# jacobkrantz/VLN-CE

Hardware: AMD Instinct MI355X
Metric: policy-steps/sec (fwd+bwd) (higher is better)
Workload: dtype f32

## Files before the change

include/vlnce_hip.h:

```cpp
#ifndef VLNCE_HIP_H
#define VLNCE_HIP_H

#include <stddef.h>
#include <stdint.h>

#ifdef __cplusplus
extern "C" {
#endif

typedef void* vlnce_stream_t;

enum { VLNCE_ACT_NONE = 0, VLNCE_ACT_RELU = 1, VLNCE_ACT_SIGMOID = 2, VLNCE_ACT_TANH = 3 };

int vlnce_version(void);
int vlnce_option_count(void);
int vlnce_option_index(const char* name);
const char* vlnce_last_error(void);

int vlnce_set_option(const char* name, int value);
int vlnce_get_option(const char* name, int* value);
int vlnce_option_default(const char* name, int* value);

typedef struct {
  int N, H, W, Cin;
  int Cout, KH, KW;
  int stride, pad;
  int Ho, Wo;
  int ldx, ldy;
} vlnce_conv_desc;

typedef struct {
  const float* x;
  int Cin, ldx;
  const void* w_frag;
  const float* in_scale;
  const float* in_shift;
  const float* in_center;
  int in_relu;
} vlnce_regen;

typedef struct {
  const float* in_scale;
  const float* in_shift;
  const float* in_center;
  int in_relu;
  const float* x2;
  const float* in2_scale;
  const float* in2_shift;
  const float* in2_center;
  float* side_out;
  const void* w_split;
  const void* w_frag;
  const int* options;
  int w_format;
  const vlnce_regen* regen;
} vlnce_prologue;

#define VLNCE_BN_SHARDS 16
typedef struct {
  double* acc;
  void* workspace;
  long workspace_bytes;
} vlnce_bn_sums;

typedef struct {
  const float* scale;
  const float* shift;
  const float* residual;
  int ldr;
  int act;
  int accumulate;
  float* stat_partial;
  const vlnce_bn_sums* bn;
  int stats_only;
} vlnce_epilogue;

long vlnce_conv2d_bn_workspace_bytes(const vlnce_conv_desc* d);
int vlnce_bn_finalize_sums(double* acc, int M, int C, const float* gamma, const float* beta,
                           float eps, float momentum, float* running_mean, float* running_var,
                           float* scale_out, float* shift_out, float* mean_out, float* rstd_out,
                           vlnce_stream_t stream);

int vlnce_conv2d_tiles_m(const vlnce_conv_desc* d);
int vlnce_conv2d_tile_rows(const vlnce_conv_desc* d);

int vlnce_conv2d_split_weights(const float* w, void* planes, long count, int format,
                               vlnce_stream_t stream);

long vlnce_conv2d_pack_bytes(const vlnce_conv_desc* d);
int vlnce_conv2d_pack_weights(const float* w_ohwi, void* frag, const vlnce_conv_desc* d,
                              int format , vlnce_stream_t stream);

typedef struct vlnce_weight_job {
  const float* w_oihw;
  void* dst;
  int Cout, Cin, T;
  int kind;
  int transposed;
  int format;
} vlnce_weight_job;
long vlnce_weight_job_items(const vlnce_weight_job* job);
int vlnce_conv2d_prepare_weights(const vlnce_weight_job* jobs_dev, const long* first_item_dev,
                                 int njobs, long total_items, vlnce_stream_t stream);

#define VLNCE_CONV_PATH_F32 0
#define VLNCE_CONV_PATH_X3 1
#define VLNCE_CONV_PATH_P3 2
#define VLNCE_CONV_PATH_M3 3
int vlnce_conv2d_last_path(void);

#define VLNCE_CONV_KERNEL(family, format, kernel, a, b, c) \
  ((family) | ((format) << 2) | ((kernel) << 4) | ((a) << 8) | ((b) << 16) | ((c) << 24))
#define VLNCE_CONV_KERNEL_FAMILY(v) ((v) & 3)
#define VLNCE_CONV_KERNEL_FORMAT(v) (((v) >> 2) & 3)
#define VLNCE_CONV_KERNEL_KIND(v) (((v) >> 4) & 15)
#define VLNCE_CONV_KERNEL_A(v) (((v) >> 8) & 255)
#define VLNCE_CONV_KERNEL_B(v) (((v) >> 16) & 255)
#define VLNCE_CONV_KERNEL_C(v) (((v) >> 24) & 127)
#define VLNCE_CONV_KERNEL_P3 0
#define VLNCE_CONV_KERNEL_U3 1
#define VLNCE_CONV_KERNEL_S3 2
#define VLNCE_CONV_KERNEL_R3 3
#define VLNCE_CONV_P3_DENSE 0
#define VLNCE_CONV_P3_GATHER 1
#define VLNCE_CONV_P3_DUAL 2
#define VLNCE_CONV_KERNEL_F32_BUF 0
#define VLNCE_CONV_KERNEL_F32_SPLITK 1
#define VLNCE_CONV_KERNEL_F32_V4 2
#define VLNCE_CONV_KERNEL_F32_S 3
#define VLNCE_CONV_KERNEL_F32_STEM3 4
#define VLNCE_CONV_KERNEL_F32_STEM1 5
#define VLNCE_CONV_KERNEL_F32_DUAL 6
int vlnce_conv2d_last_kernel(void);

int vlnce_conv2d_fwd(const float* x, const float* w_ohwi, float* y,
                     const vlnce_conv_desc* d, const vlnce_prologue* pro,
                     const vlnce_epilogue* epi, vlnce_stream_t stream);

int vlnce_gemm(const float* A, int lda, int transA, const float* B, int ldb, int transB,
               float* C, int ldc, int M, int N, int K,
               const vlnce_epilogue* epi, vlnce_stream_t stream);

#define VLNCE_GEMM_KERNEL(a, b, tile, splitk, zero, pass2) \
  ((a) | ((b) << 2) | ((tile) << 4) | ((zero) ? 1 << 6 : 0) | ((pass2) ? 1 << 7 : 0) | ((splitk) << 8))
#define VLNCE_GEMM_KERNEL_A(v) ((v) & 3)
#define VLNCE_GEMM_KERNEL_B(v) (((v) >> 2) & 3)
#define VLNCE_GEMM_KERNEL_TILE(v) (((v) >> 4) & 3)
#define VLNCE_GEMM_KERNEL_ZERO(v) (((v) >> 6) & 1)
#define VLNCE_GEMM_KERNEL_PASS2(v) (((v) >> 7) & 1)
#define VLNCE_GEMM_KERNEL_SPLITK(v) (((v) >> 8) & 255)
#define VLNCE_GEMM_A_BUF 0
#define VLNCE_GEMM_A_IM2COL_V4 1
#define VLNCE_GEMM_A_IM2COL_S 2
#define VLNCE_GEMM_A_TRANS 3
#define VLNCE_GEMM_B_BUF 0
#define VLNCE_GEMM_B_NK_V4 1
#define VLNCE_GEMM_B_NK_S 2
#define VLNCE_GEMM_B_KN 3
#define VLNCE_GEMM_TILE_128X128 1
#define VLNCE_GEMM_TILE_128X64 2
#define VLNCE_GEMM_TILE_64X64 3
int vlnce_gemm_last_kernel(void);

int vlnce_linear_rows_supported(int M, int N, int K);
int vlnce_linear_rows_fwd(const float* x, int ldx, const float* w, int ldw, const float* bias,
                          int act, float* y, int ldy, int M, int N, int K, vlnce_stream_t stream);
int vlnce_linear_rows_bwd(const float* x, int ldx, const float* w, int ldw, const float* dy,
                          int lddy, const float* y, int ldy, int act, float* dx, float* dw,
                          float* db, int M, int N, int K, vlnce_stream_t stream);

int vlnce_colsum(const float* x, int ldx, int M, int N, float* out, int accumulate,
                 vlnce_stream_t stream);

size_t vlnce_bn_finalize_workspace_bytes(int tiles_m, int C);
int vlnce_bn_finalize(const float* stat_partial, int tiles_m, int tile_rows, int M, int C,
                      const float* gamma, const float* beta, float eps, float momentum,
                      float* running_mean, float* running_var,
                      float* scale_out, float* shift_out,
                      float* mean_out, float* rstd_out,
                      void* workspace, size_t workspace_bytes,
                      vlnce_stream_t stream);

int vlnce_scale_shift_act(const float* x, const float* scale, const float* shift,
                          const float* center, int rows_per_sample, const float* residual,
                          float* y, long M, int C, int act, vlnce_stream_t stream);

int vlnce_scale_shift_add_act(const float* x1, const float* scale1, const float* shift1,
                              const float* center1, const float* x2, const float* scale2,
                              const float* shift2, const float* center2, float* y, long M, int C,
                              int act, vlnce_stream_t stream);

int vlnce_gn_chunks(int HW);
int vlnce_gn_partial(const float* x, int Nimg, int HW, int C, float* partial ,
                     vlnce_stream_t stream);
int vlnce_gn_finalize(const float* partial, int Nimg, int HW, int C, int groups,
                      const float* gamma, const float* beta, float eps,
                      float* scale_out, float* shift_out,
                      float* center_out,
                      float* mean_out, float* rstd_out,
                      vlnce_stream_t stream);
int vlnce_gn_finalize_tiles(const float* stat_partial, int tile_rows, int Nimg, int HW, int C,
                            int groups, const float* gamma, const float* beta, float eps,
                            float* scale_out, float* shift_out, float* center_out,
                            float* mean_out, float* rstd_out, vlnce_stream_t stream);
int vlnce_group_norm_small(const float* x, int Nimg, int HW, int C, int groups, const float* gamma,
                           const float* beta, float eps, const float* residual, int act, float* y,
                           vlnce_stream_t stream);

int vlnce_maxpool3x3s2(const float* x, float* y, int N, int H, int W, int C, int Ho, int Wo,
                       const float* in_scale, const float* in_shift, const float* in_center,
                       int in_relu, vlnce_stream_t stream);
int vlnce_avgpool2x2(const float* x, float* y, int N, int H, int W, int C, vlnce_stream_t stream);

int vlnce_space_to_depth2(const float* x, float* y, int N, int H, int W, int C, int pad_lo,
                          int pad_hi, const float* scale, const float* shift,
                          vlnce_stream_t stream);
#define VLNCE_DT_F32 0
#define VLNCE_DT_U8 1
typedef struct {
  const void* x;
  const void* x2;
  const unsigned char* mask2;
  int dtype;
  int N, F, Hs, Ws, C;
  int y0, x0, H, W;
} vlnce_frames;
int vlnce_frames_s2d(const vlnce_frames* frames, float* y, int pad_lo, int pad_hi,
                     const float* scale, const float* shift, vlnce_stream_t stream);
int vlnce_stem7_fwd(const vlnce_frames* frames, const float* in_scale, const float* in_shift,
                    const void* w_frag, int w_format, float* y, int Cout, const vlnce_epilogue* epi,
                    vlnce_stream_t stream);
int vlnce_frames_avgpool2(const vlnce_frames* frames, float* y, vlnce_stream_t stream);
int vlnce_frames_f32(const vlnce_frames* frames, float* y, const float* scale, const float* shift,
                     vlnce_stream_t stream);
int vlnce_frames_gather(const void* const* srcs, int F, int elem_bytes, int N, int Hs, int Ws,
                        int C, int y0, int x0, int H, int W, void* out, vlnce_stream_t stream);

int vlnce_frames_resize_area(const void* x, int dtype, int NF, int Hs, int Ws, int C, int OH, int OW,
                             int y0, int x0, int H, int W, void* out, vlnce_stream_t stream);

int vlnce_adaptive_avgpool(const float* x, float* y, int N, int H, int W, int C, int OH, int OW,
                           int ldy, vlnce_stream_t stream);

int vlnce_conv2d_wgrad(const float* x, const float* dy, float* dw_ohwi, const vlnce_conv_desc* d,
                       const float* dy_pow2, int P, int accumulate, vlnce_stream_t stream);
#define VLNCE_WGRAD_PATH_F32 0
#define VLNCE_WGRAD_PATH_X6_BF16 1
#define VLNCE_WGRAD_PATH_X6_F16 2
int vlnce_conv2d_wgrad_last_path(void);
#define VLNCE_WGRAD_KERNEL(path, tm, split) ((path) | ((tm) << 4) | ((split) ? 1 << 12 : 0))
#define VLNCE_WGRAD_KERNEL_PATH(v) ((v) & 15)
#define VLNCE_WGRAD_KERNEL_TM(v) (((v) >> 4) & 255)
#define VLNCE_WGRAD_KERNEL_SPLIT(v) (((v) >> 12) & 1)
int vlnce_conv2d_wgrad_last_kernel(void);
size_t vlnce_bn_bwd_workspace_floats(long M, int C);
int vlnce_bn_bwd(const float* dy, const float* y, const float* x, const float* mean,
                 const float* rstd, const float* gamma, long M, int C, int relu,
                 int use_batch_stats, float* dx, float* dres, float* dgamma, float* dbeta,
                 float* workspace, float* pow2, int P, vlnce_stream_t stream);
size_t vlnce_gn_bwd_workspace_floats(int Nimg, int HW, int C, int groups);
int vlnce_gn_bwd(const float* dy, const float* y, const float* x, const float* mean,
                 const float* rstd, const float* gamma, int Nimg, int HW, int C, int groups,
                 int relu, float* dx, float* dres, float* dgamma, float* dbeta, float* workspace,
                 float* pow2, int P, vlnce_stream_t stream);
int vlnce_maxpool3x3s2_argmax(const float* x, float* y, uint8_t* argmax, int N, int H, int W,
                              int C, int Ho, int Wo, vlnce_stream_t stream);
int vlnce_maxpool3x3s2_bwd(const float* dy, const uint8_t* argmax, float* dx, int N, int H, int W,
                           int C, int Ho, int Wo, vlnce_stream_t stream);
int vlnce_adaptive_avgpool_bwd(const float* dy, float* dx, int N, int H, int W, int C, int OH,
                               int OW, vlnce_stream_t stream);

int vlnce_action_head_fwd(const float* x, int ldx, const float* w, const float* b, int M, int K,
                          int A, float* logits_out, int* nan_count, vlnce_stream_t stream);
int vlnce_action_head_bwd(const float* x, int ldx, const float* w, const float* logits,
                          const float* dlogits, int M, int K, int A, float* dx, float* dw,
                          float* db, vlnce_stream_t stream);

int vlnce_attn_fwd(const float* q, const float* K, int ldk, const float* V, int ldv,
                   const uint8_t* mask, int mask_mode, float scale,
                   float* out, float* attn_out, int B, int P, int Dk, int Dv,
                   vlnce_stream_t stream);
int vlnce_attn_bwd(const float* dout, const float* q, const float* K, int ldk,
                   const float* V, int ldv, const uint8_t* mask, int mask_mode, float scale,
                   const float* attn, float* dq, float* dK, int lddk, float* dV, int lddv,
                   int B, int P, int Dk, int Dv, vlnce_stream_t stream);

int vlnce_attn_fwd_shared(const float* q, const float* K, int ldk, const float* V, int ldv,
                          const uint8_t* mask, int mask_mode, float scale, const int64_t* kv_index,
                          float* out, float* attn_out, int B, int P, int Dk, int Dv,
                          vlnce_stream_t stream);
int vlnce_attn_bwd_shared(const float* dout, const float* q, const float* K, int ldk,
                          const float* V, int ldv, const uint8_t* mask, int mask_mode, float scale,
                          const int64_t* kv_index, const float* attn, float* dq, float* dK,
                          int lddk, float* dV, int lddv, int B, int P, int Dk, int Dv,
                          vlnce_stream_t stream);
int vlnce_segment_sum(const float* x, const int64_t* index, int B, int U, long row_elems,
                      float* out, vlnce_stream_t stream);
int vlnce_rowzero_mask(const float* x, int ld, long rows, int C, uint8_t* mask,
                       vlnce_stream_t stream);

int vlnce_gru_gates_fwd(const float* gi, const float* gh, const float* h_prev,
                        const uint8_t* mask,
                        float* h_out, float* gates_out ,
                        float* hn_out ,
                        int B, int H, vlnce_stream_t stream);
int vlnce_gru_gates_bwd(const float* dh_out, const float* gates, const float* hn,
                        const float* h_prev, const uint8_t* mask,
                        float* dgi, float* dgh, float* dh_prev, int B, int H,
                        vlnce_stream_t stream);
int vlnce_lstm_gates_fwd(const float* gi, const float* gh, const float* c_prev,
                         const uint8_t* mask, float* h_out, float* c_out,
                         float* gates_out , int B, int H,
                         vlnce_stream_t stream);
int vlnce_lstm_gates_bwd(const float* dh_out, const float* dc_out, const float* gates,
                         const float* c_prev, const float* c_out, const uint8_t* mask,
                         float* dgates , float* dc_prev, int B, int H,
                         vlnce_stream_t stream);

int vlnce_rnn_seq_supported(int kind, int H);
int vlnce_rnn_seq_fwd(int kind, int dirs, const float* const* gi, const float* const* w_hh,
                      const float* const* b_hh, const int* lengths, float* const* out,
                      float* const* h_final, float* const* gates_save, float* const* aux_save,
                      int B, int L, int H, vlnce_stream_t stream);
int vlnce_rnn_seq_bwd(int kind, int dirs, const float* const* w_hh_t, const int* lengths,
                      const float* const* out, const float* const* gates_save,
                      const float* const* aux_save, const float* const* dout,
                      const float* const* dh_final, float* const* dgi, float* const* dgh,
                      int B, int L, int H, vlnce_stream_t stream);
int vlnce_rnn_seq_fwd2(int kind, int dirs, const float* const* gi, const float* const* w_hh,
                       const float* const* b_hh, const int* lengths, float* const* out_tm,
                       float* seq, long seq_st, long seq_sb, float* const* h_final,
                       float* const* gates_save, float* const* aux_save, int B, int L, int H,
                       vlnce_stream_t stream);
int vlnce_rnn_seq_bwd2(int kind, int dirs, const float* const* w_hh, const int* lengths,
                       const float* const* out_tm, const float* const* gates_save,
                       const float* const* aux_save, const float* dseq, long dseq_st, long dseq_sb,
                       float* dout_ws ,
                       const float* const* dh_final, float* const* dgi, float* const* dgh,
                       int B, int L, int H, vlnce_stream_t stream);
int vlnce_rnn_seq_wgrad(int kind, int dirs, int first_dir, const float* const* dgi, const float* const* dgh,
                        const float* const* out_tm, const float* x_tm, int ldx, int E,
                        const float* const* w_ih, float* const* dw_ih, float* const* dw_hh,
                        float* const* db_ih, float* const* db_hh, float* dx_tm, int B, int L, int H,
                        vlnce_stream_t stream);

int vlnce_mean_rows(const float* x, float* y, int B, int P, int C, vlnce_stream_t stream);
int vlnce_rnn_step_supported(int N, int H, int lstm);
int vlnce_rnn_step_fwd(int lstm, const float* gi, const float* h_prev, const float* c_prev,
                       const uint8_t* mask, const float* w_hh, const float* b_hh, float* hp_out,
                       float* h_out, float* aux_out, float* gates_out, int N, int H,
                       vlnce_stream_t stream);
int vlnce_rnn_step_bwd(int lstm, const float* dout, float* carry, const float* dc,
                       const float* gates, const float* aux, const float* hp, const float* c_prev,
                       const uint8_t* mask, const float* w_hh_t, float* dgi, float* dgh,
                       float* acc0, float* dc_prev, int N, int H, vlnce_stream_t stream);
int vlnce_mask_rows(const float* x, const uint8_t* mask, float* out, int B, int H,
                    vlnce_stream_t stream);
int vlnce_gru_rollout_supported(int N, int H);
long vlnce_gru_rollout_workspace_bytes(int N, int H);
int vlnce_gru_rollout_fwd(const float* gi, const float* h0, const uint8_t* mask, const float* w_hh,
                          const float* b_hh, float* hp, float* out, float* gates, float* aux,
                          void* workspace, int T, int N, int H, vlnce_stream_t stream);
int vlnce_gru_rollout_bwd(const float* dout, const float* dh_final, const float* gates,
                          const float* aux, const float* hp, const uint8_t* mask,
                          const float* w_hh_t, float* dgi, float* dgh, float* dh0,
                          void* workspace, int T, int N, int H, vlnce_stream_t stream);
int vlnce_lstm_rollout_supported(int N, int H);
long vlnce_lstm_rollout_workspace_bytes(int N, int H);
int vlnce_lstm_rollout_fwd(const float* gi, const float* h0, const float* c0, const uint8_t* mask,
                           const float* w_hh, const float* b_hh, float* hp, float* out, float* gates,
                           float* aux, void* workspace, int T, int N, int H, vlnce_stream_t stream);
int vlnce_lstm_rollout_bwd(const float* dout, const float* dh_final, const float* dc_final,
                           const float* gates, const float* aux, const float* hp, const float* c0,
                           const uint8_t* mask, const float* w_hh_t, float* dgi, float* dh0,
                           float* dc0, void* workspace, int T, int N, int H, vlnce_stream_t stream);

int vlnce_select_rows(const uint8_t* mask, const float* a, const float* b, float* out, int B, int H,
                      vlnce_stream_t stream);
int vlnce_embedding_bwd(const long* tokens, const float* grad_rows, float* grad_weight, long rows,
                        int E, long padding_idx, long vocab, vlnce_stream_t stream);
int vlnce_act_bwd(const float* dy, const float* y, float* dz, long n, int act,
                  vlnce_stream_t stream);

enum { VLNCE_SRC_F32 = 0, VLNCE_SRC_F16 = 1, VLNCE_SRC_I64 = 2 };
int vlnce_ragged_pad_rows(const void* src, int src_dtype, const int* offsets, int B, int Tmax,
                          long D, float fill, float* dst, vlnce_stream_t stream);
int vlnce_ragged_pad_rows_i64(const int64_t* src, const int* offsets, int B, int Tmax, long D,
                              int64_t fill, int64_t* dst, vlnce_stream_t stream);
int vlnce_dagger_targets(const int64_t* oracle_actions, const int* offsets, int B, int Tmax,
                         float inflection_coef, int64_t* corrected_out, float* weights_out,
                         uint8_t* masks_out, vlnce_stream_t stream);

enum { VLNCE_TRAJ_F32 = 0, VLNCE_TRAJ_F16 = 1, VLNCE_TRAJ_I64 = 2, VLNCE_TRAJ_U8 = 3 };
#define VLNCE_TRAJ_MAX_SENSORS 8
#define VLNCE_TRAJ_MAX_ROWS 128
typedef struct {
  const void* src;
  void* dst;
  long row_stride, c_stride, p_stride;
  int C, P;
  int src_dtype;
  int dst_dtype;
} vlnce_traj_sensor;
int vlnce_traj_append(const vlnce_traj_sensor* sensors, int n_sensors, const int* slots,
                      const int* steps, int n_rows, long capacity, vlnce_stream_t stream);
int vlnce_dagger_mix_actions(const int64_t* actions, const void* expert, int expert_dtype,
                             const float* uniform, float beta, int n, int64_t* prev_actions,
                             int64_t* stepped , vlnce_stream_t stream);

int vlnce_ppo_returns(const float* rewards, float* value_preds, const float* masks,
                      const float* next_value, float* returns, int T, int N, float gamma, float tau,
                      int use_gae, vlnce_stream_t stream);

int vlnce_ppo_loss(const float* values, const float* returns, const float* value_preds,
                   const float* logp, const float* old_logp, const float* adv,
                   const float* ent_pano, const float* ent_offset, const float* ent_distance,
                   const float* radians, int B, float clip, float value_coef, float entropy_coef,
                   float pano_coef, float offset_coef, float distance_coef, float reg_coef,
                   int use_clipped, float* stats, float* grads, vlnce_stream_t stream);

int vlnce_il_loss_supported(int T, int N, int A);
int vlnce_il_loss(const float* logits, const int64_t* targets, const float* weights,
                  const float* aux, float inv_scalar, int T, int N, int A, float* stats,
                  float* dlogits, vlnce_stream_t stream);

int vlnce_pair_mse(const float* estimate, const float* target, const uint8_t* mask, int E, int R,
                   float* value, float* d_estimate, vlnce_stream_t stream);

#ifdef __cplusplus
}
#endif
#endif
```

vln-ce_amd/_lib.py:

```python
import collections
import ctypes as C
import os
import threading

import torch

_HERE = os.path.dirname(os.path.abspath(__file__))
LIB_PATH = os.environ.get("VLNCE_HIP_LIB") or os.path.join(_HERE, "libvlnce_hip.so")

_P = C.c_void_p
_I = C.c_int
_F = C.c_float
_L = C.c_long


def _buffer_format(explicit, *bufs):
    tags = {getattr(b, "_vlnce_fmt", None) for b in bufs if b is not None} - {None}
    if explicit:
        tags.add(int(explicit))
    if len(tags) > 1:
        raise RuntimeError(f"weight buffers / w_format disagree on the plane format: {sorted(tags)}")
    return tags.pop() if tags else 1


ConvKernel = collections.namedtuple("ConvKernel", "family kernel fmt a b c")
ConvKernel.__doc__ = """family: "f32" | "x3" | "p3" | "m3" (= conv2d_last_path()); kernel: the kernel within it
("conv_p3" | "conv_u3" | "conv_s3", "conv_m3", "conv_x3", "buf" | "splitk" | "v4" | "s" | "stem3" |
"stem1" | "dual" of igemm_kernel); fmt: plane format 1 / 2 (0: fp32); a, b, c per kernel:
  conv_p3: tile 1..6, mode "dense" | "gather" | "dual", 0      conv_u3: rows, kind 0..2, waves
  conv_s3: Cin, 1 = statistics only, 0      conv_r3: regenerated Cin, Cout / 32, skip kind 1 / 2
  conv_m3: NT, KSPLIT, RB      conv_x3: tile 1..4, dual 0 / 1, 0
  splitk: the split factor, 0, 0"""
WgradKernel = collections.namedtuple("WgradKernel", "path tm split")

_FAMILIES = ("f32", "x3", "p3", "m3")
_KERNELS = {"f32": ("buf", "splitk", "v4", "s", "stem3", "stem1", "dual"), "x3": ("conv_x3",),
            "p3": ("conv_p3", "conv_u3", "conv_s3", "conv_r3"), "m3": ("conv_m3",)}
_P3_MODES = ("dense", "gather", "dual")


def decode_conv_kernel(v):
    if v < 0:
        return None
    family = _FAMILIES[v & 3]
    kernel = _KERNELS[family][(v >> 4) & 15]
    a, b, c = (v >> 8) & 255, (v >> 16) & 255, (v >> 24) & 127
    if kernel == "conv_p3":
        b = _P3_MODES[b]
    return ConvKernel(family, kernel, (v >> 2) & 3, a, b, c)


def decode_wgrad_kernel(v):
    return None if v < 0 else WgradKernel(v & 15, (v >> 4) & 255, bool((v >> 12) & 1))


GemmKernel = collections.namedtuple("GemmKernel", "a b tile splitk zero pass2")
GemmKernel.__doc__ = """a: the A loader "buf" | "v4" | "s" | "trans"; b: the B loader "buf" | "nk_v4" | "nk_s" | "kn";
tile: (rows, columns) of the igemm_kernel instance; splitk: the split-K factor (1 = not split); zero: C was
zero-filled first; pass2: the second bias / activation pass ran"""
_GEMM_A = ("buf", "v4", "s", "trans")
_GEMM_B = ("buf", "nk_v4", "nk_s", "kn")
_GEMM_TILES = (None, (128, 128), (128, 64), (64, 64))


def decode_gemm_kernel(v):
    if v < 0:
        return None
    return GemmKernel(_GEMM_A[v & 3], _GEMM_B[(v >> 2) & 3], _GEMM_TILES[(v >> 4) & 3], (v >> 8) & 255,
                      bool((v >> 6) & 1), bool((v >> 7) & 1))


class ConvDesc(C.Structure):
    _fields_ = [(n, _I) for n in
                ("N", "H", "W", "Cin", "Cout", "KH", "KW", "stride", "pad", "Ho", "Wo", "ldx", "ldy")]


class WeightJob(C.Structure):
    _fields_ = [("w_oihw", _P), ("dst", _P), ("Cout", _I), ("Cin", _I), ("T", _I), ("kind", _I),
                ("transposed", _I), ("format", _I)]


class WeightPrepPlan:
    __slots__ = ("table", "first_item", "njobs", "total", "keep")


class Prologue(C.Structure):
    _fields_ = [("in_scale", _P), ("in_shift", _P), ("in_center", _P), ("in_relu", _I),
                ("x2", _P), ("in2_scale", _P), ("in2_shift", _P), ("in2_center", _P),
                ("side_out", _P), ("w_split", _P), ("w_frag", _P), ("options", _P), ("w_format", _I),
                ("regen", _P)]


class Regen(C.Structure):
    _fields_ = [("x", _P), ("Cin", _I), ("ldx", _I), ("w_frag", _P), ("in_scale", _P), ("in_shift", _P),
                ("in_center", _P), ("in_relu", _I)]


class Frames(C.Structure):
    _fields_ = [("x", _P), ("x2", _P), ("mask2", _P), ("dtype", _I), ("N", _I), ("F", _I),
                ("Hs", _I), ("Ws", _I), ("C", _I), ("y0", _I), ("x0", _I), ("H", _I), ("W", _I)]


class BnSums(C.Structure):
    _fields_ = [("acc", _P), ("workspace", _P), ("workspace_bytes", _L)]


class TrajSensor(C.Structure):
    _fields_ = [("src", _P), ("dst", _P), ("row_stride", _L), ("c_stride", _L), ("p_stride", _L),
                ("C", _I), ("P", _I), ("src_dtype", _I), ("dst_dtype", _I)]


class Epilogue(C.Structure):
    _fields_ = [("scale", _P), ("shift", _P), ("residual", _P), ("ldr", _I), ("act", _I),
                ("accumulate", _I), ("stat_partial", _P), ("bn", C.POINTER(BnSums)),
                ("stats_only", _I)]


_SIGNATURES = {
    "vlnce_version": (_I, []),
    "vlnce_last_error": (C.c_char_p, []),
    "vlnce_set_option": (_I, [C.c_char_p, _I]),
    "vlnce_get_option": (_I, [C.c_char_p, C.POINTER(_I)]),
    "vlnce_option_default": (_I, [C.c_char_p, C.POINTER(_I)]),
    "vlnce_conv2d_split_weights": (_I, [_P, _P, C.c_long, _I, _P]),
    "vlnce_conv2d_last_path": (_I, []),
    "vlnce_conv2d_wgrad_last_path": (_I, []),
    "vlnce_conv2d_last_kernel": (_I, []),
    "vlnce_conv2d_wgrad_last_kernel": (_I, []),
    "vlnce_gemm_last_kernel": (_I, []),
    "vlnce_embedding_bwd": (_I, [_P, _P, _P, _L, _I, _L, _L, _P]),
    "vlnce_conv2d_pack_bytes": (C.c_long, [C.POINTER(ConvDesc)]),
    "vlnce_conv2d_pack_weights": (_I, [_P, _P, C.POINTER(ConvDesc), _I, _P]),
    "vlnce_weight_job_items": (C.c_long, [C.POINTER(WeightJob)]),
    "vlnce_conv2d_prepare_weights": (_I, [_P, _P, _I, C.c_long, _P]),
    "vlnce_conv2d_tiles_m": (_I, [C.POINTER(ConvDesc)]),
    "vlnce_conv2d_tile_rows": (_I, [C.POINTER(ConvDesc)]),
    "vlnce_conv2d_bn_workspace_bytes": (C.c_long, [C.POINTER(ConvDesc)]),
    "vlnce_bn_finalize_sums": (_I, [_P, _I, _I, _P, _P, _F, _F, _P, _P, _P, _P, _P, _P, _P]),
    "vlnce_conv2d_fwd": (_I, [_P, _P, _P, C.POINTER(ConvDesc), C.POINTER(Prologue),
                              C.POINTER(Epilogue), _P]),
    "vlnce_gemm": (_I, [_P, _I, _I, _P, _I, _I, _P, _I, _I, _I, _I, C.POINTER(Epilogue), _P]),
    "vlnce_colsum": (_I, [_P, _I, _I, _I, _P, _I, _P]),
    "vlnce_bn_finalize_workspace_bytes": (C.c_size_t, [_I, _I]),
    "vlnce_bn_finalize": (_I, [_P, _I, _I, _I, _I, _P, _P, _F, _F, _P, _P, _P, _P, _P, _P, _P,
                               C.c_size_t, _P]),
    "vlnce_scale_shift_act": (_I, [_P, _P, _P, _P, _I, _P, _P, _L, _I, _I, _P]),
    "vlnce_gn_chunks": (_I, [_I]),
    "vlnce_gn_partial": (_I, [_P, _I, _I, _I, _P, _P]),
    "vlnce_gn_finalize": (_I, [_P, _I, _I, _I, _I, _P, _P, _F, _P, _P, _P, _P, _P, _P]),
    "vlnce_gn_finalize_tiles": (_I, [_P, _I, _I, _I, _I, _I, _P, _P, _F, _P, _P, _P, _P, _P, _P]),
    "vlnce_maxpool3x3s2": (_I, [_P, _P, _I, _I, _I, _I, _I, _I, _P, _P, _P, _I, _P]),
    "vlnce_scale_shift_add_act": (_I, [_P, _P, _P, _P, _P, _P, _P, _P, _P, _L, _I, _I, _P]),
    "vlnce_avgpool2x2": (_I, [_P, _P, _I, _I, _I, _I, _P]),
    "vlnce_ragged_pad_rows": (_I, [_P, _I, _P, _I, _I, _L, _F, _P, _P]),
    "vlnce_ragged_pad_rows_i64": (_I, [_P, _P, _I, _I, _L, _L, _P, _P]),
    "vlnce_dagger_targets": (_I, [_P, _P, _I, _I, _F, _P, _P, _P, _P]),
    "vlnce_traj_append": (_I, [C.POINTER(TrajSensor), _I, C.POINTER(_I), C.POINTER(_I), _I, _L, _P]),
    "vlnce_dagger_mix_actions": (_I, [_P, _P, _I, _P, _F, _I, _P, _P, _P]),
    "vlnce_ppo_loss": (_I, [_P, _P, _P, _P, _P, _P, _P, _P, _P, _P, _I, _F, _F, _F, _F, _F, _F, _F, _I,
                            _P, _P, _P]),
    "vlnce_ppo_returns": (_I, [_P, _P, _P, _P, _P, _I, _I, _F, _F, _I, _P]),
    "vlnce_il_loss_supported": (_I, [_I, _I, _I]),
    "vlnce_il_loss": (_I, [_P, _P, _P, _P, _F, _I, _I, _I, _P, _P, _P]),
    "vlnce_pair_mse": (_I, [_P, _P, _P, _I, _I, _P, _P, _P]),
    "vlnce_space_to_depth2": (_I, [_P, _P, _I, _I, _I, _I, _I, _I, _P, _P, _P]),
    "vlnce_frames_s2d": (_I, [C.POINTER(Frames), _P, _I, _I, _P, _P, _P]),
    "vlnce_frames_avgpool2": (_I, [C.POINTER(Frames), _P, _P]),
    "vlnce_stem7_fwd": (_I, [C.POINTER(Frames), _P, _P, _P, _I, _P, _I, C.POINTER(Epilogue), _P]),
    "vlnce_frames_f32": (_I, [C.POINTER(Frames), _P, _P, _P, _P]),
    "vlnce_frames_gather": (_I, [_P, _I, _I, _I, _I, _I, _I, _I, _I, _I, _I, _P, _P]),
    "vlnce_frames_resize_area": (_I, [_P] + [_I] * 11 + [_P, _P]),
    "vlnce_adaptive_avgpool": (_I, [_P, _P, _I, _I, _I, _I, _I, _I, _I, _P]),
    "vlnce_attn_fwd": (_I, [_P, _P, _I, _P, _I, _P, _I, _F, _P, _P, _I, _I, _I, _I, _P]),
    "vlnce_attn_bwd": (_I, [_P, _P, _P, _I, _P, _I, _P, _I, _F, _P, _P, _P, _I, _P, _I,
                            _I, _I, _I, _I, _P]),
    "vlnce_rowzero_mask": (_I, [_P, _I, _L, _I, _P, _P]),
    "vlnce_attn_fwd_shared": (_I, [_P, _P, _I, _P, _I, _P, _I, _F, _P, _P, _P, _I, _I, _I, _I, _P]),
    "vlnce_attn_bwd_shared": (_I, [_P, _P, _P, _I, _P, _I, _P, _I, _F, _P, _P, _P, _P, _I, _P, _I,
                                   _I, _I, _I, _I, _P]),
    "vlnce_segment_sum": (_I, [_P, _P, _I, _I, _L, _P, _P]),
    "vlnce_action_head_fwd": (_I, [_P, _I, _P, _P, _I, _I, _I, _P, _P, _P]),
    "vlnce_action_head_bwd": (_I, [_P, _I, _P, _P, _P, _I, _I, _I, _P, _P, _P, _P]),
    "vlnce_gru_gates_fwd": (_I, [_P, _P, _P, _P, _P, _P, _P, _I, _I, _P]),
    "vlnce_gru_gates_bwd": (_I, [_P, _P, _P, _P, _P, _P, _P, _P, _I, _I, _P]),
    "vlnce_lstm_gates_fwd": (_I, [_P, _P, _P, _P, _P, _P, _P, _I, _I, _P]),
    "vlnce_lstm_gates_bwd": (_I, [_P, _P, _P, _P, _P, _P, _P, _P, _I, _I, _P]),
    "vlnce_mean_rows": (_I, [_P, _P, _I, _I, _I, _P]),
    "vlnce_mask_rows": (_I, [_P, _P, _P, _I, _I, _P]),
    "vlnce_conv2d_wgrad": (_I, [_P, _P, _P, C.POINTER(ConvDesc), _P, _I, _I, _P]),
    "vlnce_bn_bwd": (_I, [_P, _P, _P, _P, _P, _P, _L, _I, _I, _I, _P, _P, _P, _P, _P, _P, _I, _P]),
    "vlnce_bn_bwd_workspace_floats": (C.c_size_t, [_L, _I]),
    "vlnce_gn_bwd_workspace_floats": (C.c_size_t, [_I, _I, _I, _I]),
    "vlnce_gn_bwd": (_I, [_P, _P, _P, _P, _P, _P, _I, _I, _I, _I, _I, _P, _P, _P, _P, _P, _P, _I, _P]),
    "vlnce_maxpool3x3s2_argmax": (_I, [_P, _P, _P, _I, _I, _I, _I, _I, _I, _P]),
    "vlnce_maxpool3x3s2_bwd": (_I, [_P, _P, _P, _I, _I, _I, _I, _I, _I, _P]),
    "vlnce_adaptive_avgpool_bwd": (_I, [_P, _P, _I, _I, _I, _I, _I, _I, _P]),
    "vlnce_rnn_seq_supported": (_I, [_I, _I]),
    "vlnce_rnn_seq_fwd": (_I, [_I, _I, _P, _P, _P, _P, _P, _P, _P, _P, _I, _I, _I, _P]),
    "vlnce_rnn_seq_bwd": (_I, [_I, _I, _P, _P, _P, _P, _P, _P, _P, _P, _P, _I, _I, _I, _P]),
    "vlnce_option_count": (_I, []),
    "vlnce_option_index": (_I, [C.c_char_p]),
    "vlnce_linear_rows_supported": (_I, [_I, _I, _I]),
    "vlnce_linear_rows_fwd": (_I, [_P, _I, _P, _I, _P, _I, _P, _I, _I, _I, _I, _P]),
    "vlnce_linear_rows_bwd": (_I, [_P, _I, _P, _I, _P, _I, _P, _I, _I, _P, _P, _P, _I, _I, _I, _P]),
    "vlnce_rnn_seq_fwd2": (_I, [_I, _I, _P, _P, _P, _P, _P, _P, _L, _L, _P, _P, _P, _I, _I, _I, _P]),
    "vlnce_rnn_seq_bwd2": (_I, [_I, _I, _P, _P, _P, _P, _P, _P, _L, _L, _P, _P, _P, _P, _I, _I, _I, _P]),
    "vlnce_rnn_seq_wgrad": (_I, [_I, _I, _I, _P, _P, _P, _P, _I, _I, _P, _P, _P, _P, _P, _P, _I, _I, _I, _P]),
    "vlnce_group_norm_small": (_I, [_P, _I, _I, _I, _I, _P, _P, _F, _P, _I, _P, _P]),
    "vlnce_gru_rollout_supported": (_I, [_I, _I]),
    "vlnce_gru_rollout_workspace_bytes": (C.c_long, [_I, _I]),
    "vlnce_gru_rollout_fwd": (_I, [_P, _P, _P, _P, _P, _P, _P, _P, _P, _P, _I, _I, _I, _P]),
    "vlnce_gru_rollout_bwd": (_I, [_P, _P, _P, _P, _P, _P, _P, _P, _P, _P, _P, _I, _I, _I, _P]),
    "vlnce_lstm_rollout_supported": (_I, [_I, _I]),
    "vlnce_lstm_rollout_workspace_bytes": (C.c_long, [_I, _I]),
    "vlnce_lstm_rollout_fwd": (_I, [_P, _P, _P, _P, _P, _P, _P, _P, _P, _P, _P, _I, _I, _I, _P]),
    "vlnce_lstm_rollout_bwd": (_I, [_P, _P, _P, _P, _P, _P, _P, _P, _P, _P, _P, _P, _P, _I, _I, _I, _P]),
    "vlnce_rnn_step_supported": (_I, [_I, _I, _I]),
    "vlnce_rnn_step_fwd": (_I, [_I, _P, _P, _P, _P, _P, _P, _P, _P, _P, _P, _I, _I, _P]),
    "vlnce_rnn_step_bwd": (_I, [_I, _P, _P, _P, _P, _P, _P, _P, _P, _P, _P, _P, _P, _P, _I, _I, _P]),
    "vlnce_select_rows": (_I, [_P, _P, _P, _P, _I, _I, _P]),
    "vlnce_act_bwd": (_I, [_P, _P, _P, _L, _I, _P]),
}


def collapse_rows(t):
    while True:
        groups = []
        for n, st in zip(t.shape[1:], t.stride()[1:]):
            if n == 1:
                continue
            if groups and groups[-1][1] == st * n:
                groups[-1] = (groups[-1][0] * n, int(st))
            else:
                groups.append((int(n), int(st)))
        if len(groups) <= 2:
            break
        t = t.contiguous()
    row_stride = int(t.stride(0)) if t.size(0) > 1 else 0
    if not groups:
        return t, row_stride, 1, 0, 1, 0
    if len(groups) == 1:
        return t, row_stride, groups[0][0], groups[0][1], 1, 0
    return t, row_stride, groups[0][0], groups[0][1], groups[1][0], groups[1][1]


def exported_symbols():
    return sorted(_SIGNATURES)


def load_cdll(path=LIB_PATH):
    if not os.path.exists(path):
        raise RuntimeError(
            f"{path} not found: build it with `python __graft_entry__.py` (hipcc, gfx950). "
            "The VLN-CE policy path has no CPU fallback."
        )
    dll = C.CDLL(path)
    for name, (res, args) in _SIGNATURES.items():
        fn = getattr(dll, name)
        fn.restype = res
        fn.argtypes = args
    return dll


class _CallState(threading.local):
    dev = None
    restore = None


_CALL = _CallState()


def _ptr(t):
    if t is None:
        return None
    if not t.is_cuda:
        raise RuntimeError("libvlnce_hip: tensor is not on a GPU (no CPU fallback)")
    idx = t.device.index
    if _CALL.dev is None:
        _CALL.dev = idx
    elif _CALL.dev != idx:
        first, _CALL.dev = _CALL.dev, None
        raise RuntimeError(f"libvlnce_hip: tensors of one call live on cuda:{first} and "
                           f"cuda:{idx}")
    return t.data_ptr()


def _stream():
    dev, _CALL.dev = _CALL.dev, None
    if dev is None:
        return torch.cuda.current_stream().cuda_stream
    cur = torch.cuda.current_device()
    if dev != cur:
        _CALL.restore = cur
        torch.cuda.set_device(dev)
    return torch.cuda.current_stream(dev).cuda_stream


def _leave_device():
    if _CALL.restore is not None:
        cur, _CALL.restore = _CALL.restore, None
        torch.cuda.set_device(cur)


class HipLib:

    name = "hip"

    ABI = 150

    def __init__(self, path=LIB_PATH):
        self.dll = load_cdll(path)
        have = int(self.dll.vlnce_version())
        if have != self.ABI:
            raise RuntimeError(f"{path} has ABI {have}, this package binds ABI {self.ABI}: "
                               "rebuild it (python __graft_entry__.py)")

        self._conv_math = None
        self._tls = threading.local()
        self._options_from_env()

    OPTION_NAMES = ("conv_math", "p3", "p3_tile", "s3", "u3", "u3_waves", "x3_tile", "igemm_tile",
                    "igemm_nobuf", "igemm_no_splitk", "wgrad_tile", "rollout_one_xcd", "m3", "r3",
                    "s3_wgs")

    def _options_from_env(self):
        for name in self.OPTION_NAMES:
            v = os.environ.get("VLNCE_" + name.upper())
            if v is None:
                continue
            if name == "conv_math":
                v = {"f32": 0, "0": 0, "bf16": 1, "1": 1, "f16": 2, "2": 2}.get(v.strip().lower(), v)
            elif name in ("igemm_nobuf", "igemm_no_splitk"):
                v = 0 if v in ("", "0") else 1
            try:
                v = int(v)
            except ValueError:
                import warnings
                warnings.warn(f"VLNCE_{name.upper()}={v!r} is not an integer: ignored "
                              f"(the option keeps its default)")
                continue
            self.set_option(name, v)

    def set_option(self, name, value):
        self._check(self.dll.vlnce_set_option(name.encode(), int(value)), "vlnce_set_option")
        if name == "conv_math":
            self._conv_math = int(value)

    def plane_format(self, options=None):
        v = None
        if options:
            v = options.get("conv_math")
        if v is None:
            sc = getattr(self._tls, "scoped", None)
            if sc:
                v = sc.get("conv_math")
        if v is None or v < 0:
            v = self._conv_math
            if v is None:
                v = self._conv_math = self.get_option("conv_math")
        return 2 if v == 2 else 1

    def effective_option(self, name):
        sc = getattr(self._tls, "scoped", None)
        if sc and sc.get(name, -1) >= 0:
            return int(sc[name])
        return self.get_option(name)

    def get_option(self, name):
        v = _I(0)
        self._check(self.dll.vlnce_get_option(name.encode(), C.byref(v)), "vlnce_get_option")
        return v.value

    def option_default(self, name):
        v = _I(0)
        self._check(self.dll.vlnce_option_default(name.encode(), C.byref(v)), "vlnce_option_default")
        return v.value

    PER_LAUNCH = ("conv_math", "p3", "p3_tile", "s3", "u3", "u3_waves", "x3_tile", "m3", "r3", "s3_wgs")

    def _launch_options(self, overrides):
        if not overrides:
            return None
        arr = (C.c_int * int(self.dll.vlnce_option_count()))(*([-1] * int(self.dll.vlnce_option_count())))
        for name, v in overrides.items():
            i = int(self.dll.vlnce_option_index(name.encode()))
            if i < 0:
                raise RuntimeError(f"unknown dispatch option {name!r}")
            arr[i] = int(v)
        return arr

    def options(self, **kw):
        lib = self
        unknown = [k for k in kw if k not in self.OPTION_NAMES]
        if unknown:
            raise RuntimeError(f"unknown dispatch option(s) {unknown}")

        class _Scope:
            def __enter__(self_inner):
                self_inner.prev = getattr(lib._tls, "scoped", None)
                scoped = dict(self_inner.prev or {})
                scoped.update({k: v for k, v in kw.items() if k in lib.PER_LAUNCH})
                lib._tls.scoped = scoped or None
                self_inner.old = {k: lib.get_option(k) for k in kw if k not in lib.PER_LAUNCH}
                for k in self_inner.old:
                    lib.set_option(k, kw[k])
                return lib

            def __exit__(self_inner, *exc):
                lib._tls.scoped = self_inner.prev
                for k, v in self_inner.old.items():
                    lib.set_option(k, v)
                return False

        return _Scope()

    def _check(self, rc, what):
        _leave_device()
        if rc != 0:
            raise RuntimeError(f"{what} failed (rc={rc}): {self.dll.vlnce_last_error().decode()}")

    @staticmethod
    def _desc(g):
        return ConvDesc(*[int(g[k]) for k, _ in ConvDesc._fields_])

    def conv2d_tiles(self, g):
        d = self._desc(g)
        return self.dll.vlnce_conv2d_tiles_m(C.byref(d)), self.dll.vlnce_conv2d_tile_rows(C.byref(d))

    def conv2d_fwd(self, x, w, y, g, in_scale=None, in_shift=None, in_relu=0, scale=None,
                   shift=None, residual=None, ldr=0, act=0, accumulate=0, stat_partial=None,
                   in_center=None, x2=None, in2_scale=None, in2_shift=None, in2_center=None,
                   side_out=None, w_split=None, w_frag=None, bn=None, options=None, w_format=None,
                   stats_only=False, regen=None):
        d = self._desc(g)
        w_format = _buffer_format(w_format, w_split, w_frag, regen["w_frag"] if regen else None)
        rg = None
        if regen is not None:
            rx = regen["x"]
            rg = Regen(_ptr(rx), rx.size(-1), rx.size(-1), _ptr(regen["w_frag"]),
                       _ptr(regen.get("in_scale")), _ptr(regen.get("in_shift")),
                       _ptr(regen.get("in_center")), int(regen.get("in_relu", 0)))
        opts = self._launch_options(options if options is not None
                                    else getattr(self._tls, "scoped", None))
        pro = Prologue(_ptr(in_scale), _ptr(in_shift), _ptr(in_center), int(in_relu), _ptr(x2),
                       _ptr(in2_scale), _ptr(in2_shift), _ptr(in2_center), _ptr(side_out),
                       _ptr(w_split), _ptr(w_frag),
                       C.cast(opts, C.c_void_p) if opts is not None else None, int(w_format),
                       C.cast(C.pointer(rg), C.c_void_p) if rg is not None else None)
        bnp = None
        if bn is not None:
            acc, ws = bn
            bnp = C.pointer(BnSums(_ptr(acc), _ptr(ws), ws.numel() * ws.element_size()))
        epi = Epilogue(_ptr(scale), _ptr(shift), _ptr(residual), int(ldr), int(act),
                       int(accumulate), _ptr(stat_partial), bnp, int(bool(stats_only)))
        self._check(self.dll.vlnce_conv2d_fwd(_ptr(x), _ptr(w), _ptr(y), C.byref(d), C.byref(pro),
                                              C.byref(epi), _stream()), "vlnce_conv2d_fwd")

    def bn_finalize_sums(self, acc, M, gamma, beta, eps, momentum, running_mean, running_var,
                         scale_out, mean_out, shift_out=None, rstd_out=None):
        Cc = scale_out.numel()
        self._check(self.dll.vlnce_bn_finalize_sums(
            _ptr(acc), int(M), Cc, _ptr(gamma), _ptr(beta), float(eps), float(momentum),
            _ptr(running_mean), _ptr(running_var), _ptr(scale_out), _ptr(shift_out),
            _ptr(mean_out), _ptr(rstd_out), _stream()), "vlnce_bn_finalize_sums")

    def conv2d_bn_workspace_bytes(self, g):
        d = self._desc(g)
        return int(self.dll.vlnce_conv2d_bn_workspace_bytes(C.byref(d)))

    def conv2d_split_weights(self, w, planes, fmt=1):
        self._check(self.dll.vlnce_conv2d_split_weights(_ptr(w), _ptr(planes), w.numel(), int(fmt),
                                                        _stream()), "vlnce_conv2d_split_weights")

    def conv2d_last_path(self):
        return int(self.dll.vlnce_conv2d_last_path())

    def conv2d_wgrad_last_path(self):
        return int(self.dll.vlnce_conv2d_wgrad_last_path())

    def conv2d_last_kernel(self):
        return decode_conv_kernel(int(self.dll.vlnce_conv2d_last_kernel()))

    def conv2d_wgrad_last_kernel(self):
        return decode_wgrad_kernel(int(self.dll.vlnce_conv2d_wgrad_last_kernel()))

    def conv2d_pack_bytes(self, g):
        d = self._desc(g)
        return int(self.dll.vlnce_conv2d_pack_bytes(C.byref(d)))

    def conv2d_pack_weights(self, w, frag, g, fmt=1):
        d = self._desc(g)
        self._check(self.dll.vlnce_conv2d_pack_weights(_ptr(w), _ptr(frag), C.byref(d), int(fmt),
                                                       _stream()), "vlnce_conv2d_pack_weights")

    WP_F32, WP_PLANES, WP_FRAGMENTS = 0, 1, 2

    def weight_prep_plan(self, jobs):
        arr = (WeightJob * len(jobs))()
        first = [0]
        for j, (w, dst, kind, transposed, fmt) in zip(arr, jobs):
            assert w.is_cuda and w.is_contiguous() and w.dtype == torch.float32 and w.dim() == 4
            j.w_oihw, j.dst = w.data_ptr(), dst.data_ptr()
            j.Cout, j.Cin, j.T = w.size(0), w.size(1), w.size(2) * w.size(3)
            j.kind, j.transposed, j.format = int(kind), int(bool(transposed)), int(fmt or 0)
            items = int(self.dll.vlnce_weight_job_items(C.byref(j)))
            if items <= 0:
                raise ValueError(f"weight_prep_plan: job not eligible: {tuple(w.shape)} kind={kind} "
                                 f"transposed={transposed} format={fmt}")
            first.append(first[-1] + items)
        plan = WeightPrepPlan()
        dev = jobs[0][1].device
        plan.table = torch.frombuffer(bytearray(bytes(arr)), dtype=torch.uint8).to(dev)
        plan.first_item = torch.tensor(first, dtype=torch.int64).to(dev)
        plan.njobs, plan.total = len(jobs), first[-1]
        plan.keep = [(w, dst) for w, dst, *_ in jobs]
        return plan

    def conv2d_prepare_weights(self, plan):
        self._check(self.dll.vlnce_conv2d_prepare_weights(_ptr(plan.table), _ptr(plan.first_item),
                                                          plan.njobs, plan.total, _stream()),
                    "vlnce_conv2d_prepare_weights")

    def gemm(self, A, lda, transA, B, ldb, transB, Cm, ldc, M, N, K, scale=None, shift=None,
             residual=None, ldr=0, act=0, accumulate=0):
        epi = Epilogue(_ptr(scale), _ptr(shift), _ptr(residual), int(ldr), int(act),
                       int(accumulate), None)
        self._check(self.dll.vlnce_gemm(_ptr(A), lda, transA, _ptr(B), ldb, transB, _ptr(Cm), ldc,
                                        M, N, K, C.byref(epi), _stream()), "vlnce_gemm")

    def gemm_last_kernel(self):
        return decode_gemm_kernel(int(self.dll.vlnce_gemm_last_kernel()))

    def colsum(self, x, ldx, M, N, out, accumulate=0):
        self._check(self.dll.vlnce_colsum(_ptr(x), ldx, M, N, _ptr(out), accumulate, _stream()),
                    "vlnce_colsum")

    def bn_finalize_workspace_bytes(self, tiles_m, Cc):
        return int(self.dll.vlnce_bn_finalize_workspace_bytes(tiles_m, Cc))

    def bn_finalize(self, partial, tiles_m, tile_rows, M, Cc, gamma, beta, eps, momentum,
                    running_mean, running_var, scale_out, shift_out, mean_out=None, rstd_out=None,
                    workspace=None):
        wb = workspace.numel() * workspace.element_size() if workspace is not None else 0
        self._check(self.dll.vlnce_bn_finalize(
            _ptr(partial), tiles_m, tile_rows, M, Cc, _ptr(gamma), _ptr(beta), eps, momentum,
            _ptr(running_mean), _ptr(running_var), _ptr(scale_out), _ptr(shift_out),
            _ptr(mean_out), _ptr(rstd_out), _ptr(workspace), wb, _stream()), "vlnce_bn_finalize")

    def scale_shift_act(self, x, scale, shift, rows_per_sample, residual, y, M, Cc, act,
                        center=None):
        self._check(self.dll.vlnce_scale_shift_act(
            _ptr(x), _ptr(scale), _ptr(shift), _ptr(center), rows_per_sample, _ptr(residual),
            _ptr(y), M, Cc, act, _stream()), "vlnce_scale_shift_act")

    def gn_chunks(self, HW):
        return self.dll.vlnce_gn_chunks(HW)

    def gn_partial(self, x, Nimg, HW, Cc, partial):
        self._check(self.dll.vlnce_gn_partial(_ptr(x), Nimg, HW, Cc, _ptr(partial), _stream()),
                    "vlnce_gn_partial")

    def gn_finalize(self, partial, Nimg, HW, Cc, groups, gamma, beta, eps, scale_out, shift_out,
                    mean_out=None, rstd_out=None, center_out=None):
        self._check(self.dll.vlnce_gn_finalize(
            _ptr(partial), Nimg, HW, Cc, groups, _ptr(gamma), _ptr(beta), eps, _ptr(scale_out),
            _ptr(shift_out), _ptr(center_out), _ptr(mean_out), _ptr(rstd_out), _stream()),
            "vlnce_gn_finalize")

    def gn_finalize_tiles(self, partial, tile_rows, Nimg, HW, Cc, groups, gamma, beta, eps,
                          scale_out, shift_out, mean_out=None, rstd_out=None, center_out=None):
        self._check(self.dll.vlnce_gn_finalize_tiles(
            _ptr(partial), tile_rows, Nimg, HW, Cc, groups, _ptr(gamma), _ptr(beta), eps,
            _ptr(scale_out), _ptr(shift_out), _ptr(center_out), _ptr(mean_out), _ptr(rstd_out),
            _stream()), "vlnce_gn_finalize_tiles")

    def maxpool3x3s2(self, x, y, N, H, W, Cc, Ho, Wo, in_scale=None, in_shift=None, in_relu=0,
                     in_center=None):
        self._check(self.dll.vlnce_maxpool3x3s2(_ptr(x), _ptr(y), N, H, W, Cc, Ho, Wo,
                                                _ptr(in_scale), _ptr(in_shift), _ptr(in_center),
                                                int(in_relu), _stream()), "vlnce_maxpool3x3s2")

    def scale_shift_add_act(self, x1, s1, t1, x2, s2, t2, y, M, Cc, act, c1=None, c2=None):
        self._check(self.dll.vlnce_scale_shift_add_act(
            _ptr(x1), _ptr(s1), _ptr(t1), _ptr(c1), _ptr(x2), _ptr(s2), _ptr(t2), _ptr(c2),
            _ptr(y), M, Cc, act, _stream()), "vlnce_scale_shift_add_act")

    _SRC = {torch.float32: 0, torch.float16: 1, torch.int64: 2}

    def ragged_pad_rows(self, src, offsets, B, Tmax, D, fill, dst):
        assert offsets.dtype == torch.int32 and dst.dtype == torch.float32
        self._check(self.dll.vlnce_ragged_pad_rows(
            _ptr(src), self._SRC[src.dtype], _ptr(offsets), B, Tmax, D, float(fill),
            _ptr(dst), _stream()), "vlnce_ragged_pad_rows")

    def ragged_pad_rows_i64(self, src, offsets, B, Tmax, D, fill, dst):
        assert src.dtype == torch.int64 and dst.dtype == torch.int64
        self._check(self.dll.vlnce_ragged_pad_rows_i64(
            _ptr(src), _ptr(offsets), B, Tmax, D, int(fill), _ptr(dst), _stream()),
            "vlnce_ragged_pad_rows_i64")

    def dagger_targets(self, oracle, offsets, B, Tmax, coef, corrected, weights, masks):
        self._check(self.dll.vlnce_dagger_targets(
            _ptr(oracle), _ptr(offsets), B, Tmax, float(coef), _ptr(corrected),
            _ptr(weights), _ptr(masks), _stream()), "vlnce_dagger_targets")

    _TRAJ = {torch.float32: 0, torch.float16: 1, torch.int64: 2, torch.uint8: 3}
    TRAJ_MAX_SENSORS, TRAJ_MAX_ROWS = 8, 128

    def traj_append(self, sources, arenas, slots, steps):
        n = len(slots)
        assert len(sources) == len(arenas) and len(steps) == n and n > 0
        capacity, num_envs = int(arenas[0].size(1)), min(int(a.size(0)) for a in arenas)
        if min(slots) < 0 or max(slots) >= num_envs:
            raise RuntimeError(f"traj_append: slot outside the arena's {num_envs} environments")
        table, keep = [], []
        for src, dst in zip(sources, arenas):
            src, rs, Cc, cs, P, ps = collapse_rows(src)
            keep.append(src)
            if src.size(0) != n:
                raise RuntimeError(f"traj_append: {src.size(0)} source rows for {n} slots")
            if dst.dim() != 3 or not dst.is_contiguous() or dst.size(1) != capacity \
                    or dst.size(2) != Cc * P:
                raise RuntimeError(f"traj_append: arena {tuple(dst.shape)} for rows of {Cc * P} "
                                   f"elements at capacity {capacity}")
            if src.dtype not in (torch.float32, torch.int64, torch.uint8) \
                    or dst.dtype not in (torch.float16, torch.float32, torch.int64):
                raise RuntimeError(f"traj_append: {src.dtype} -> {dst.dtype} is not a recorded pair")
            table.append((src, dst, rs, Cc, cs, P, ps))
        for r0 in range(0, n, self.TRAJ_MAX_ROWS):
            r1 = min(n, r0 + self.TRAJ_MAX_ROWS)
            sl = (_I * (r1 - r0))(*[int(v) for v in slots[r0:r1]])
            stp = (_I * (r1 - r0))(*[int(v) for v in steps[r0:r1]])
            for k0 in range(0, len(table), self.TRAJ_MAX_SENSORS):
                part = table[k0:k0 + self.TRAJ_MAX_SENSORS]
                arr = (TrajSensor * len(part))()
                for a, (src, dst, rs, Cc, cs, P, ps) in zip(arr, part):
                    a.src = _ptr(src) + r0 * rs * src.element_size()
                    a.dst = _ptr(dst)
                    a.row_stride, a.c_stride, a.p_stride, a.C, a.P = rs, cs, ps, Cc, P
                    a.src_dtype, a.dst_dtype = self._TRAJ[src.dtype], self._TRAJ[dst.dtype]
                self._check(self.dll.vlnce_traj_append(arr, len(part), sl, stp, r1 - r0, capacity,
                                                       _stream()), "vlnce_traj_append")

    def dagger_mix_actions(self, actions, expert, uniform, beta, prev_actions, stepped):
        n = actions.numel()
        assert actions.dtype == torch.int64 and prev_actions.dtype == torch.int64
        assert stepped.dtype == torch.int64 and stepped.numel() == 2 * n and stepped.is_contiguous()
        assert uniform.dtype == torch.float32 and expert.dtype in (torch.float32, torch.int64)
        assert expert.numel() == n and uniform.numel() == n and prev_actions.numel() == n
        assert all(t.is_contiguous() for t in (actions, expert, uniform, prev_actions))
        self._check(self.dll.vlnce_dagger_mix_actions(
            _ptr(actions), _ptr(expert), self._TRAJ[expert.dtype], _ptr(uniform), float(beta), n,
            _ptr(prev_actions), _ptr(stepped), _stream()), "vlnce_dagger_mix_actions")

    def ppo_loss(self, values, returns, value_preds, logp, old_logp, adv, ent_pano, ent_offset,
                 ent_distance, radians, B, clip, value_coef, entropy_coef, pano_coef, offset_coef,
                 distance_coef, reg_coef, use_clipped, stats, grads):
        self._check(self.dll.vlnce_ppo_loss(
            _ptr(values), _ptr(returns), _ptr(value_preds), _ptr(logp), _ptr(old_logp), _ptr(adv),
            _ptr(ent_pano), _ptr(ent_offset), _ptr(ent_distance), _ptr(radians), B, clip, value_coef,
            entropy_coef, pano_coef, offset_coef, distance_coef, reg_coef, int(use_clipped),
            _ptr(stats), _ptr(grads), _stream()), "vlnce_ppo_loss")

    def ppo_returns(self, rewards, value_preds, masks, next_value, returns, T, N, gamma, tau,
                    use_gae):
        self._check(self.dll.vlnce_ppo_returns(_ptr(rewards), _ptr(value_preds), _ptr(masks),
                                               _ptr(next_value), _ptr(returns), T, N, float(gamma),
                                               float(tau), int(use_gae), _stream()),
                    "vlnce_ppo_returns")

    def il_loss_supported(self, T, N, A):
        return bool(self.dll.vlnce_il_loss_supported(int(T), int(N), int(A)))

    def il_loss(self, logits, targets, weights, aux, inv_scalar, T, N, A, stats, dlogits):
        assert logits.dtype == torch.float32 and weights.dtype == torch.float32
        assert targets.dtype == torch.int64 and (aux is None or aux.dtype == torch.float32)
        assert logits.numel() == T * N * A and targets.numel() == T * N and weights.numel() == T * N
        assert stats.numel() == 3 and dlogits.numel() == T * N * A
        assert all(t.is_contiguous() for t in (logits, targets, weights, stats, dlogits))
        self._check(self.dll.vlnce_il_loss(_ptr(logits), _ptr(targets), _ptr(weights), _ptr(aux),
                                           float(inv_scalar), T, N, A, _ptr(stats), _ptr(dlogits),
                                           _stream()), "vlnce_il_loss")

    def pair_mse(self, estimate, target, mask, E, R, value, d_estimate):
        assert estimate.dtype == torch.float32 and target.dtype == torch.float32
        assert mask.dtype in (torch.bool, torch.uint8) and mask.numel() == E
        assert estimate.numel() == E and target.numel() == R and d_estimate.numel() == E
        assert all(t.is_contiguous() for t in (estimate, target, mask, d_estimate))
        self._check(self.dll.vlnce_pair_mse(_ptr(estimate), _ptr(target), _ptr(mask), E, R,
                                            _ptr(value), _ptr(d_estimate), _stream()),
                    "vlnce_pair_mse")

    def space_to_depth2(self, x, y, N, H, W, Cc, pad_lo, pad_hi, scale=None, shift=None):
        self._check(self.dll.vlnce_space_to_depth2(_ptr(x), _ptr(y), N, H, W, Cc, pad_lo, pad_hi,
                                                   _ptr(scale), _ptr(shift), _stream()),
                    "vlnce_space_to_depth2")

    _DT = {torch.float32: 0, torch.uint8: 1}

    def _frames(self, fr):
        x = fr["x"]
        if fr.get("x2") is not None and fr["x2"].dtype != x.dtype:
            raise RuntimeError("libvlnce_hip: frames and the extra frame differ in dtype")
        return Frames(_ptr(x), _ptr(fr.get("x2")), _ptr(fr.get("mask2")), self._DT[x.dtype],
                      *[int(fr[k]) for k in ("N", "F", "Hs", "Ws", "C", "y0", "x0", "H", "W")])

    def frames_s2d(self, fr, y, pad_lo, pad_hi, scale=None, shift=None):
        d = self._frames(fr)
        self._check(self.dll.vlnce_frames_s2d(C.byref(d), _ptr(y), pad_lo, pad_hi, _ptr(scale),
                                              _ptr(shift), _stream()), "vlnce_frames_s2d")

    def stem7_fwd(self, fr, in_scale, in_shift, w_frag, y, scale=None, shift=None, act=0, bn=None,
                  w_format=None):
        d = self._frames(fr)
        w_format = _buffer_format(w_format, w_frag)
        bnp = None
        if bn is not None:
            bnp = C.pointer(BnSums(_ptr(bn), None, 0))
        epi = Epilogue(_ptr(scale), _ptr(shift), None, 0, int(act), 0, None, bnp)
        self._check(self.dll.vlnce_stem7_fwd(C.byref(d), _ptr(in_scale), _ptr(in_shift),
                                             _ptr(w_frag), int(w_format), _ptr(y), y.size(-1),
                                             C.byref(epi), _stream()), "vlnce_stem7_fwd")

    def frames_avgpool2(self, fr, y):
        d = self._frames(fr)
        self._check(self.dll.vlnce_frames_avgpool2(C.byref(d), _ptr(y), _stream()),
                    "vlnce_frames_avgpool2")

    def frames_f32(self, fr, y, scale=None, shift=None):
        d = self._frames(fr)
        self._check(self.dll.vlnce_frames_f32(C.byref(d), _ptr(y), _ptr(scale), _ptr(shift),
                                              _stream()), "vlnce_frames_f32")

    def frames_gather(self, srcs, elem_bytes, N, Hs, Ws, Cc, y0, x0, H, W, out):
        arr = (C.c_void_p * len(srcs))(*[_ptr(t) for t in srcs])
        self._check(self.dll.vlnce_frames_gather(arr, len(srcs), elem_bytes, N, Hs, Ws, Cc, y0, x0,
                                                 H, W, _ptr(out), _stream()), "vlnce_frames_gather")

    def frames_resize_area(self, x, is_u8, NF, Hs, Ws, Cc, OH, OW, y0, x0, H, W, out):
        self._check(self.dll.vlnce_frames_resize_area(_ptr(x), 1 if is_u8 else 0, NF, Hs, Ws, Cc, OH,
                                                      OW, y0, x0, H, W, _ptr(out), _stream()),
                    "vlnce_frames_resize_area")

    def avgpool2x2(self, x, y, N, H, W, Cc):
        self._check(self.dll.vlnce_avgpool2x2(_ptr(x), _ptr(y), N, H, W, Cc, _stream()),
                    "vlnce_avgpool2x2")

    def adaptive_avgpool(self, x, y, N, H, W, Cc, OH, OW, ldy):
        self._check(self.dll.vlnce_adaptive_avgpool(_ptr(x), _ptr(y), N, H, W, Cc, OH, OW, ldy,
                                                    _stream()), "vlnce_adaptive_avgpool")

    def mean_rows(self, x, y, B, P, Cc):
        self._check(self.dll.vlnce_mean_rows(_ptr(x), _ptr(y), B, P, Cc, _stream()),
                    "vlnce_mean_rows")

    def action_head_fwd(self, x, ldx, w, b, M, K, A, logits_out, nan_count=None):
        self._check(self.dll.vlnce_action_head_fwd(_ptr(x), ldx, _ptr(w), _ptr(b), M, K, A,
                                                   _ptr(logits_out), _ptr(nan_count), _stream()),
                    "vlnce_action_head_fwd")

    def action_head_bwd(self, x, ldx, w, logits, dlogits, M, K, A, dx=None, dw=None, db=None):
        self._check(self.dll.vlnce_action_head_bwd(_ptr(x), ldx, _ptr(w), _ptr(logits),
                                                   _ptr(dlogits), M, K, A, _ptr(dx), _ptr(dw),
                                                   _ptr(db), _stream()), "vlnce_action_head_bwd")

    def attn_fwd(self, q, K, ldk, V, ldv, mask, mask_mode, scale, out, attn_out, B, P, Dk, Dv,
                 kv_index=None):
        if kv_index is not None:
            self._check(self.dll.vlnce_attn_fwd_shared(
                _ptr(q), _ptr(K), ldk, _ptr(V), ldv, _ptr(mask), mask_mode, scale, _ptr(kv_index),
                _ptr(out), _ptr(attn_out), B, P, Dk, Dv, _stream()), "vlnce_attn_fwd_shared")
            return
        self._check(self.dll.vlnce_attn_fwd(_ptr(q), _ptr(K), ldk, _ptr(V), ldv, _ptr(mask),
                                            mask_mode, scale, _ptr(out), _ptr(attn_out), B, P, Dk,
                                            Dv, _stream()), "vlnce_attn_fwd")

    def segment_sum(self, x, index, B, U, row_elems, out):
        self._check(self.dll.vlnce_segment_sum(_ptr(x), _ptr(index), B, U, row_elems, _ptr(out),
                                               _stream()), "vlnce_segment_sum")

    def attn_bwd(self, dout, q, K, ldk, V, ldv, mask, mask_mode, scale, attn, dq, dK, lddk, dV,
                 lddv, B, P, Dk, Dv, kv_index=None):
        if kv_index is not None:
            self._check(self.dll.vlnce_attn_bwd_shared(
                _ptr(dout), _ptr(q), _ptr(K), ldk, _ptr(V), ldv, _ptr(mask), mask_mode, scale,
                _ptr(kv_index), _ptr(attn), _ptr(dq), _ptr(dK), lddk, _ptr(dV), lddv, B, P, Dk, Dv,
                _stream()), "vlnce_attn_bwd_shared")
            return
        self._check(self.dll.vlnce_attn_bwd(_ptr(dout), _ptr(q), _ptr(K), ldk, _ptr(V), ldv,
                                            _ptr(mask), mask_mode, scale, _ptr(attn), _ptr(dq),
                                            _ptr(dK), lddk, _ptr(dV), lddv, B, P, Dk, Dv,
                                            _stream()), "vlnce_attn_bwd")

    def rowzero_mask(self, x, ld, rows, Cc, mask):
        self._check(self.dll.vlnce_rowzero_mask(_ptr(x), ld, rows, Cc, _ptr(mask), _stream()),
                    "vlnce_rowzero_mask")

    def gru_gates_fwd(self, gi, gh, h_prev, mask, h_out, gates_out, hn_out, B, H):
        self._check(self.dll.vlnce_gru_gates_fwd(_ptr(gi), _ptr(gh), _ptr(h_prev), _ptr(mask),
                                                 _ptr(h_out), _ptr(gates_out), _ptr(hn_out), B, H,
                                                 _stream()), "vlnce_gru_gates_fwd")

    def gru_gates_bwd(self, dh_out, gates, hn, h_prev, mask, dgi, dgh, dh_prev, B, H):
        self._check(self.dll.vlnce_gru_gates_bwd(_ptr(dh_out), _ptr(gates), _ptr(hn), _ptr(h_prev),
                                                 _ptr(mask), _ptr(dgi), _ptr(dgh), _ptr(dh_prev),
                                                 B, H, _stream()), "vlnce_gru_gates_bwd")

    def lstm_gates_fwd(self, gi, gh, c_prev, mask, h_out, c_out, gates_out, B, H):
        self._check(self.dll.vlnce_lstm_gates_fwd(_ptr(gi), _ptr(gh), _ptr(c_prev), _ptr(mask),
                                                  _ptr(h_out), _ptr(c_out), _ptr(gates_out), B, H,
                                                  _stream()), "vlnce_lstm_gates_fwd")

    def lstm_gates_bwd(self, dh_out, dc_out, gates, c_prev, c_out, mask, dgates, dc_prev, B, H):
        self._check(self.dll.vlnce_lstm_gates_bwd(_ptr(dh_out), _ptr(dc_out), _ptr(gates),
                                                  _ptr(c_prev), _ptr(c_out), _ptr(mask),
                                                  _ptr(dgates), _ptr(dc_prev), B, H, _stream()),
                    "vlnce_lstm_gates_bwd")

    def mask_rows(self, x, mask, out, B, H):
        self._check(self.dll.vlnce_mask_rows(_ptr(x), _ptr(mask), _ptr(out), B, H, _stream()),
                    "vlnce_mask_rows")

    def conv2d_wgrad(self, x, dy, dw, g, dy_pow2=None, accumulate=False):
        d = self._desc(g)
        self._check(self.dll.vlnce_conv2d_wgrad(_ptr(x), _ptr(dy), _ptr(dw), C.byref(d),
                                                _ptr(dy_pow2),
                                                dy_pow2.size(1) if dy_pow2 is not None else 0,
                                                int(bool(accumulate)), _stream()),
                    "vlnce_conv2d_wgrad")

    def bn_bwd_workspace_floats(self, M, Cc):
        return int(self.dll.vlnce_bn_bwd_workspace_floats(M, Cc))

    def bn_bwd(self, dy, y, x, mean, rstd, gamma, M, Cc, relu, use_batch_stats, dx, dres, dgamma,
               dbeta, workspace=None, pow2=None):
        self._check(self.dll.vlnce_bn_bwd(_ptr(dy), _ptr(y), _ptr(x), _ptr(mean), _ptr(rstd),
                                          _ptr(gamma), M, Cc, int(relu), int(use_batch_stats),
                                          _ptr(dx), _ptr(dres), _ptr(dgamma), _ptr(dbeta),
                                          _ptr(workspace), _ptr(pow2),
                                          pow2.size(1) if pow2 is not None else 0, _stream()),
                    "vlnce_bn_bwd")

    def gn_bwd_workspace_floats(self, Nimg, HW, Cc, groups):
        return int(self.dll.vlnce_gn_bwd_workspace_floats(Nimg, HW, Cc, groups))

    def gn_bwd(self, dy, y, x, mean, rstd, gamma, Nimg, HW, Cc, groups, relu, dx, dres, dgamma,
               dbeta, workspace, pow2=None):
        self._check(self.dll.vlnce_gn_bwd(_ptr(dy), _ptr(y), _ptr(x), _ptr(mean), _ptr(rstd),
                                          _ptr(gamma), Nimg, HW, Cc, groups, int(relu), _ptr(dx),
                                          _ptr(dres), _ptr(dgamma), _ptr(dbeta), _ptr(workspace),
                                          _ptr(pow2), pow2.size(1) if pow2 is not None else 0,
                                          _stream()), "vlnce_gn_bwd")

    def maxpool3x3s2_argmax(self, x, y, argmax, N, H, W, Cc, Ho, Wo):
        self._check(self.dll.vlnce_maxpool3x3s2_argmax(_ptr(x), _ptr(y), _ptr(argmax), N, H, W, Cc,
                                                       Ho, Wo, _stream()),
                    "vlnce_maxpool3x3s2_argmax")

    def maxpool3x3s2_bwd(self, dy, argmax, dx, N, H, W, Cc, Ho, Wo):
        self._check(self.dll.vlnce_maxpool3x3s2_bwd(_ptr(dy), _ptr(argmax), _ptr(dx), N, H, W, Cc,
                                                    Ho, Wo, _stream()), "vlnce_maxpool3x3s2_bwd")

    def adaptive_avgpool_bwd(self, dy, dx, N, H, W, Cc, OH, OW):
        self._check(self.dll.vlnce_adaptive_avgpool_bwd(_ptr(dy), _ptr(dx), N, H, W, Cc, OH, OW,
                                                        _stream()), "vlnce_adaptive_avgpool_bwd")

    @staticmethod
    def _parr(ts, n):
        if ts is None:
            return None
        arr = (C.c_void_p * 2)()
        for i in range(n):
            arr[i] = _ptr(ts[i])
        return arr

    def rnn_seq_supported(self, kind, H):
        return bool(self.dll.vlnce_rnn_seq_supported(kind, H))

    def rnn_seq_fwd(self, kind, dirs, gi, w_hh, b_hh, lengths, out, h_final, gates_save, aux_save,
                    B, Lm, H):
        pa = self._parr
        self._check(self.dll.vlnce_rnn_seq_fwd(
            kind, dirs, pa(gi, dirs), pa(w_hh, dirs), pa(b_hh, dirs), _ptr(lengths), pa(out, dirs),
            pa(h_final, dirs), pa(gates_save, dirs), pa(aux_save, dirs), B, Lm, H, _stream()),
            "vlnce_rnn_seq_fwd")

    def rnn_seq_bwd(self, kind, dirs, w_hh_t, lengths, out, gates_save, aux_save, dout, dh_final,
                    dgi, dgh, B, Lm, H):
        pa = self._parr
        self._check(self.dll.vlnce_rnn_seq_bwd(
            kind, dirs, pa(w_hh_t, dirs), _ptr(lengths), pa(out, dirs), pa(gates_save, dirs),
            pa(aux_save, dirs), pa(dout, dirs), pa(dh_final, dirs), pa(dgi, dirs), pa(dgh, dirs),
            B, Lm, H, _stream()), "vlnce_rnn_seq_bwd")

    def linear_rows_supported(self, M, N, K):
        return bool(self.dll.vlnce_linear_rows_supported(M, N, K))

    def linear_rows_fwd(self, x, ldx, w, ldw, bias, act, y, ldy, M, N, K):
        self._check(self.dll.vlnce_linear_rows_fwd(_ptr(x), ldx, _ptr(w), ldw, _ptr(bias), act, _ptr(y),
                                                   ldy, M, N, K, _stream()), "vlnce_linear_rows_fwd")

    def linear_rows_bwd(self, x, ldx, w, ldw, dy, lddy, y, ldy, act, dx, dw, db, M, N, K):
        self._check(self.dll.vlnce_linear_rows_bwd(_ptr(x), ldx, _ptr(w), ldw, _ptr(dy), lddy, _ptr(y),
                                                   ldy, act, _ptr(dx), _ptr(dw), _ptr(db), M, N, K,
                                                   _stream()), "vlnce_linear_rows_bwd")

    def rnn_seq_fwd2(self, kind, dirs, gi, w_hh, b_hh, lengths, out_tm, seq, seq_st, seq_sb, h_final,
                     gates_save, aux_save, B, Lm, H):
        pa = self._parr
        self._check(self.dll.vlnce_rnn_seq_fwd2(
            kind, dirs, pa(gi, dirs), pa(w_hh, dirs), pa(b_hh, dirs), _ptr(lengths), pa(out_tm, dirs),
            _ptr(seq), seq_st, seq_sb, pa(h_final, dirs), pa(gates_save, dirs), pa(aux_save, dirs),
            B, Lm, H, _stream()), "vlnce_rnn_seq_fwd2")

    def rnn_seq_bwd2(self, kind, dirs, w_hh, lengths, out_tm, gates_save, aux_save, dseq, dseq_st,
                     dseq_sb, dout_ws, dh_final, dgi, dgh, B, Lm, H):
        pa = self._parr
        self._check(self.dll.vlnce_rnn_seq_bwd2(
            kind, dirs, pa(w_hh, dirs), _ptr(lengths), pa(out_tm, dirs), pa(gates_save, dirs),
            pa(aux_save, dirs), _ptr(dseq), dseq_st, dseq_sb, _ptr(dout_ws), pa(dh_final, dirs),
            pa(dgi, dirs), pa(dgh, dirs), B, Lm, H, _stream()), "vlnce_rnn_seq_bwd2")

    def rnn_seq_wgrad(self, kind, dirs, dgi, dgh, out_tm, x_tm, ldx, E, w_ih, dw_ih, dw_hh, db_ih,
                      db_hh, dx_tm, B, Lm, H, first_dir=0):
        pa = self._parr
        self._check(self.dll.vlnce_rnn_seq_wgrad(
            kind, dirs, first_dir, pa(dgi, dirs), pa(dgh, dirs), pa(out_tm, dirs), _ptr(x_tm), ldx, E,
            pa(w_ih, dirs), pa(dw_ih, dirs), pa(dw_hh, dirs), pa(db_ih, dirs), pa(db_hh, dirs),
            _ptr(dx_tm), B, Lm, H, _stream()), "vlnce_rnn_seq_wgrad")

    def group_norm_small(self, x, N, HW, Cc, groups, gamma, beta, eps, residual, act, y):
        self._check(self.dll.vlnce_group_norm_small(
            _ptr(x), N, HW, Cc, groups, _ptr(gamma), _ptr(beta), eps, _ptr(residual), act, _ptr(y),
            _stream()), "vlnce_group_norm_small")

    def gru_rollout_supported(self, N, H):
        if os.environ.get("VLNCE_GRU_ROLLOUT", "1") == "0":
            return False
        return bool(self.dll.vlnce_gru_rollout_supported(N, H))

    def gru_rollout_workspace_bytes(self, N, H):
        return int(self.dll.vlnce_gru_rollout_workspace_bytes(N, H))

    def gru_rollout_fwd(self, gi, h0, mask, w_hh, b_hh, hp, out, gates, aux, workspace, T, N, H):
        self._check(self.dll.vlnce_gru_rollout_fwd(
            _ptr(gi), _ptr(h0), _ptr(mask), _ptr(w_hh), _ptr(b_hh), _ptr(hp), _ptr(out),
            _ptr(gates), _ptr(aux), _ptr(workspace), T, N, H, _stream()), "vlnce_gru_rollout_fwd")

    def gru_rollout_bwd(self, dout, dh_final, gates, aux, hp, mask, w_hh_t, dgi, dgh, dh0,
                        workspace, T, N, H):
        self._check(self.dll.vlnce_gru_rollout_bwd(
            _ptr(dout), _ptr(dh_final), _ptr(gates), _ptr(aux), _ptr(hp), _ptr(mask),
            _ptr(w_hh_t), _ptr(dgi), _ptr(dgh), _ptr(dh0), _ptr(workspace), T, N, H, _stream()),
            "vlnce_gru_rollout_bwd")

    def lstm_rollout_supported(self, N, H):
        return bool(self.dll.vlnce_lstm_rollout_supported(N, H))

    def lstm_rollout_workspace_bytes(self, N, H):
        return int(self.dll.vlnce_lstm_rollout_workspace_bytes(N, H))

    def lstm_rollout_fwd(self, gi, h0, c0, mask, w_hh, b_hh, hp, out, gates, aux, workspace,
                         T, N, H):
        self._check(self.dll.vlnce_lstm_rollout_fwd(
            _ptr(gi), _ptr(h0), _ptr(c0), _ptr(mask), _ptr(w_hh), _ptr(b_hh), _ptr(hp), _ptr(out),
            _ptr(gates), _ptr(aux), _ptr(workspace), T, N, H, _stream()), "vlnce_lstm_rollout_fwd")

    def lstm_rollout_bwd(self, dout, dh_final, dc_final, gates, aux, hp, c0, mask, w_hh_t, dgi,
                         dh0, dc0, workspace, T, N, H):
        self._check(self.dll.vlnce_lstm_rollout_bwd(
            _ptr(dout), _ptr(dh_final), _ptr(dc_final), _ptr(gates), _ptr(aux), _ptr(hp), _ptr(c0),
            _ptr(mask), _ptr(w_hh_t), _ptr(dgi), _ptr(dh0), _ptr(dc0), _ptr(workspace), T, N, H,
            _stream()), "vlnce_lstm_rollout_bwd")

    def rnn_step_supported(self, N, H, lstm):
        if os.environ.get("VLNCE_RNN_STEP_FUSED", "1") == "0":
            return False
        return bool(self.dll.vlnce_rnn_step_supported(N, H, int(lstm)))

    def rnn_step_fwd(self, lstm, gi, h_prev, c_prev, mask, w_hh, b_hh, hp_out, h_out, aux_out,
                     gates_out, N, H):
        self._check(self.dll.vlnce_rnn_step_fwd(
            int(lstm), _ptr(gi), _ptr(h_prev), _ptr(c_prev), _ptr(mask), _ptr(w_hh), _ptr(b_hh),
            _ptr(hp_out), _ptr(h_out), _ptr(aux_out), _ptr(gates_out), N, H, _stream()),
            "vlnce_rnn_step_fwd")

    def rnn_step_bwd(self, lstm, dout, carry, dc, gates, aux, hp, c_prev, mask, w_hh_t, dgi, dgh,
                     acc0, dc_prev, N, H):
        self._check(self.dll.vlnce_rnn_step_bwd(
            int(lstm), _ptr(dout), _ptr(carry), _ptr(dc), _ptr(gates), _ptr(aux), _ptr(hp),
            _ptr(c_prev), _ptr(mask), _ptr(w_hh_t), _ptr(dgi), _ptr(dgh), _ptr(acc0),
            _ptr(dc_prev), N, H, _stream()), "vlnce_rnn_step_bwd")

    def select_rows(self, mask, a, b, out, B, H):
        self._check(self.dll.vlnce_select_rows(_ptr(mask), _ptr(a), _ptr(b), _ptr(out), B, H,
                                               _stream()), "vlnce_select_rows")

    def embedding_bwd(self, tokens, grad_rows, grad_weight, padding_idx):
        self._check(self.dll.vlnce_embedding_bwd(_ptr(tokens), _ptr(grad_rows), _ptr(grad_weight),
                                                 tokens.numel(), grad_weight.size(1),
                                                 -1 if padding_idx is None else int(padding_idx),
                                                 grad_weight.size(0), _stream()),
                    "vlnce_embedding_bwd")

    def act_bwd(self, dy, y, dz, n, act):
        self._check(self.dll.vlnce_act_bwd(_ptr(dy), _ptr(y), _ptr(dz), n, act, _stream()),
                    "vlnce_act_bwd")


_LIB = None


def get_lib():
    global _LIB
    if _LIB is None:
        _LIB = HipLib()
    return _LIB
```

vln-ce_amd/csrc/api.cpp:

```cpp
#include <stdarg.h>
#include <stdio.h>
#include <string.h>

#include <atomic>

#include "common_opts.h"

static thread_local char g_err[512] = "";

void vlnce_set_error(const char* fmt, ...) {
  va_list ap;
  va_start(ap, fmt);
  vsnprintf(g_err, sizeof(g_err), fmt, ap);
  va_end(ap);
}

extern "C" const char* vlnce_last_error(void) { return g_err; }
extern "C" int vlnce_version(void) { return 150; }

namespace {
struct OptDef {
  const char* name;
  int def;
};
const OptDef kOpts[VLNCE_OPT_COUNT] = {
    {"conv_math", 2},   {"p3", 2},          {"p3_tile", 0},         {"s3", 1},
    {"u3", 1},          {"u3_waves", 8},    {"x3_tile", 0},         {"igemm_tile", 0},
    {"igemm_nobuf", 0}, {"igemm_no_splitk", 0}, {"wgrad_tile", 64}, {"rollout_one_xcd", 0},
    {"m3", 1},          {"r3", 1},          {"s3_wgs", 0},
};
std::atomic<int> g_opt[VLNCE_OPT_COUNT] = {
    {2}, {2}, {0}, {1}, {1}, {8}, {0}, {0}, {0}, {0}, {64}, {0}, {1}, {1}, {0},
};
int opt_index(const char* name) {
  if (name)
    for (int i = 0; i < VLNCE_OPT_COUNT; ++i)
      if (strcmp(name, kOpts[i].name) == 0) return i;
  return -1;
}
}

namespace {
thread_local const int* t_call_opts = nullptr;
}
VlnceOptScope::VlnceOptScope(const int* per_call) : prev(t_call_opts) { t_call_opts = per_call; }
VlnceOptScope::~VlnceOptScope() { t_call_opts = prev; }

int vlnce_opt(int id) {
  if (t_call_opts && t_call_opts[id] >= 0) return t_call_opts[id];
  return g_opt[id].load(std::memory_order_relaxed);
}

extern "C" int vlnce_option_count(void) { return VLNCE_OPT_COUNT; }

extern "C" int vlnce_option_index(const char* name) { return opt_index(name); }

extern "C" int vlnce_set_option(const char* name, int value) {
  const int i = opt_index(name);
  if (i < 0) {
    vlnce_set_error("vlnce_set_option: unknown option '%s'", name ? name : "(null)");
    return 1;
  }
  g_opt[i].store(value, std::memory_order_relaxed);
  return 0;
}

extern "C" int vlnce_get_option(const char* name, int* value) {
  const int i = opt_index(name);
  if (i < 0 || !value) {
    vlnce_set_error("vlnce_get_option: unknown option '%s'", name ? name : "(null)");
    return 1;
  }
  *value = g_opt[i].load(std::memory_order_relaxed);
  return 0;
}

extern "C" int vlnce_option_default(const char* name, int* value) {
  const int i = opt_index(name);
  if (i < 0 || !value) {
    vlnce_set_error("vlnce_option_default: unknown option '%s'", name ? name : "(null)");
    return 1;
  }
  *value = kOpts[i].def;
  return 0;
}
```

vln-ce_amd/csrc/common_opts.h:

```cpp
#pragma once
#include "../../include/vlnce_hip.h"

void vlnce_set_error(const char* fmt, ...);

enum {
  VLNCE_OPT_CONV_MATH,
  VLNCE_OPT_P3,
  VLNCE_OPT_P3_TILE,
  VLNCE_OPT_S3,
  VLNCE_OPT_U3,
  VLNCE_OPT_U3_WAVES,
  VLNCE_OPT_X3_TILE,
  VLNCE_OPT_IGEMM_TILE,
  VLNCE_OPT_IGEMM_NOBUF,
  VLNCE_OPT_IGEMM_NO_SPLITK,
  VLNCE_OPT_WGRAD_TILE,
  VLNCE_OPT_ROLLOUT_ONE_XCD,
  VLNCE_OPT_M3,
  VLNCE_OPT_R3,
  VLNCE_OPT_S3_WGS,
  VLNCE_OPT_COUNT
};
int vlnce_opt(int id);

struct VlnceOptScope {
  explicit VlnceOptScope(const int* per_call);
  ~VlnceOptScope();
  const int* prev;
};
```

vln-ce_amd/csrc/rnn_seq.hip:

```cpp
#include "common.h"

namespace {

struct RnnSeqParams {
  const float* gi[2];
  const float* w_hh[2];
  const float* b_hh[2];
  float* out[2];
  float* h_final[2];
  float* gates[2];
  float* aux[2];
  const float* dout[2];
  const float* dh_final[2];
  float* dgi[2];
  float* dgh[2];
  const int* lengths;
  int B, L;
  float* seq[2];
  long seq_st, seq_sb;
  int self_zero;
  int w_plain;
};

__global__ __launch_bounds__(256) void dseq_to_time_major_kernel(const float* __restrict__ dseq, long st,
                                                                 long sb, float* __restrict__ dst, int dirs,
                                                                 int L, int B, int H) {
  const int h4 = H / 4;
  const long n = (long)dirs * L * B * h4;
  for (long i = (long)blockIdx.x * 256 + threadIdx.x; i < n; i += (long)gridDim.x * 256) {
    const int u4 = (int)(i % h4);
    long r = i / h4;
    const int b = (int)(r % B);
    r /= B;
    const int t = (int)(r % L);
    const int d = (int)(r / L);
    const float* src = dseq + (long)t * st + (long)b * sb + d * H + 4 * u4;
    f32x4 v = {src[0], src[1], src[2], src[3]};
    *reinterpret_cast<f32x4*>(dst + i * 4) = v;
  }
}

template <int NT>
__device__ __forceinline__ void zero_tails(float* __restrict__ base, long st, long sb, int width,
                                           const int* __restrict__ lengths, int b0, int B, int L,
                                           int tid) {
  for (int r = 0; r < 16; ++r) {
    const int b = b0 + r;
    if (b >= B) break;
    const int lb = min(max(lengths[b], 0), L);
    const int n = (L - lb) * width;
    for (int i = tid; i < n; i += NT) {
      const int q = i / width;
      base[(long)(lb + q) * st + (long)b * sb + (i - q * width)] = 0.f;
    }
  }
}

__device__ __forceinline__ float sigm(float x) {
  return __builtin_amdgcn_rcpf(1.f + __builtin_amdgcn_exp2f(-1.4426950408889634f * x));
}
__device__ __forceinline__ float tanh_fast(float x) {
  return 1.f - 2.f * __builtin_amdgcn_rcpf(__builtin_amdgcn_exp2f(2.8853900817779268f * x) + 1.f);
}

typedef __bf16 bf16x8 __attribute__((ext_vector_type(8)));
typedef unsigned u32x4r __attribute__((ext_vector_type(4)));
struct Planes3 {
  bf16x8 p[3];
};
__device__ __forceinline__ Planes3 split_planes(f32x4 lo4, f32x4 hi4) {
  const float x[8] = {lo4[0], lo4[1], lo4[2], lo4[3], hi4[0], hi4[1], hi4[2], hi4[3]};
  u32x4r h, m, l;
#pragma unroll
  for (int q = 0; q < 4; ++q) {
    const float x0 = x[2 * q], x1 = x[2 * q + 1];
    const float r0 = x0 - __uint_as_float(__float_as_uint(x0) & 0xffff0000u);
    const float r1 = x1 - __uint_as_float(__float_as_uint(x1) & 0xffff0000u);
    const float s0 = r0 - __uint_as_float(__float_as_uint(r0) & 0xffff0000u);
    const float s1 = r1 - __uint_as_float(__float_as_uint(r1) & 0xffff0000u);
    h[q] = __builtin_amdgcn_perm(__float_as_uint(x1), __float_as_uint(x0), 0x07060302u);
    m[q] = __builtin_amdgcn_perm(__float_as_uint(r1), __float_as_uint(r0), 0x07060302u);
    l[q] = __builtin_amdgcn_perm(__float_as_uint(s1), __float_as_uint(s0), 0x07060302u);
  }
  Planes3 o;
  o.p[0] = __builtin_bit_cast(bf16x8, h);
  o.p[1] = __builtin_bit_cast(bf16x8, m);
  o.p[2] = __builtin_bit_cast(bf16x8, l);
  return o;
}
__device__ __forceinline__ void split_scalar(float x, unsigned short (&o)[3]) {
  const unsigned xb = __float_as_uint(x);
  const float r = x - __uint_as_float(xb & 0xffff0000u);
  const unsigned rb = __float_as_uint(r);
  const float t = r - __uint_as_float(rb & 0xffff0000u);
  o[0] = (unsigned short)(xb >> 16);
  o[1] = (unsigned short)(rb >> 16);
  o[2] = (unsigned short)(__float_as_uint(t) >> 16);
}
constexpr int X3_PA[6] = {2, 0, 1, 1, 0, 0};
constexpr int X3_PB[6] = {0, 2, 1, 0, 1, 0};

template <int KIND, int H, int NW>
__global__ __launch_bounds__(NW * 64) void rnn_seq_fwd_kernel(RnnSeqParams p) {
  constexpr int G = KIND == 0 ? 4 : 3;
  constexpr int NTW = H / (NW * 16);
  static_assert(NTW >= 1, "units per wave");
  constexpr int KS = H / 32;
  constexpr int LDHB = H + 16;
  __shared__ __attribute__((aligned(16))) unsigned short h_pl[2][3][16][LDHB];
  constexpr int KL = (KIND == 0 && H == 128) ? 3 : 0;
  __shared__ __attribute__((aligned(16))) bf16x8 w_lds[KL > 0 ? KL : 1][3][NW * 64];
  const int d = blockIdx.y;
  const int b0 = blockIdx.x * 16;
  const int tid = threadIdx.x, lane = tid & 63, wave = tid >> 6;
  const int l15 = lane & 15, quad = lane >> 4;
  const bool reverse = d == 1;
  const float* __restrict__ gi = p.gi[d];
  const float* __restrict__ W = p.w_hh[d];
  const int B = p.B, L = p.L;
  if (p.self_zero) {
    zero_tails<NW * 64>(p.out[d], (long)B * H, H, H, p.lengths, b0, B, L, tid);
    if (p.seq[d]) zero_tails<NW * 64>(p.seq[d], p.seq_st, p.seq_sb, H, p.lengths, b0, B, L, tid);
  }

  int len[4];
#pragma unroll
  for (int r = 0; r < 4; ++r) {
    const int b = b0 + quad * 4 + r;
    len[r] = b < B ? p.lengths[b] : 0;
  }
  int Lt = max(max(len[0], len[1]), max(len[2], len[3]));
  Lt = max(Lt, __shfl_xor(Lt, 16, 64));
  Lt = max(Lt, __shfl_xor(Lt, 32, 64));
  Lt = min(Lt, L);
  Planes3 wp[G][NTW][KS];
  float bias[G][NTW];
#pragma unroll
  for (int gt = 0; gt < G; ++gt)
#pragma unroll
    for (int nt = 0; nt < NTW; ++nt) {
      const int n = gt * H + wave * (H / NW) + nt * 16 + l15;
      bias[gt][nt] = p.b_hh[d][n];
#pragma unroll
      for (int ks = 0; ks < KS; ++ks) {
        const float* w8 = W + (long)n * H + 32 * ks + 8 * quad;
        wp[gt][nt][ks] = split_planes(*reinterpret_cast<const f32x4*>(w8),
                                      *reinterpret_cast<const f32x4*>(w8 + 4));
        if (KL > 0 && gt == G - 1 && nt == 0 && ks >= KS - KL) {
#pragma unroll
          for (int q = 0; q < 3; ++q) w_lds[ks - (KS - KL)][q][tid] = wp[gt][nt][ks].p[q];
        }
      }
    }
  float hreg[NTW][4], creg[NTW][4];
#pragma unroll
  for (int nt = 0; nt < NTW; ++nt)
#pragma unroll
    for (int r = 0; r < 4; ++r) hreg[nt][r] = creg[nt][r] = 0.f;
  for (int i = tid; i < 3 * 16 * LDHB; i += NW * 64) (&h_pl[0][0][0][0])[i] = 0;
  __syncthreads();

  float gx[G][NTW][4];
  auto fetch_into = [&](int s, float (&dst)[G][NTW][4]) {
#pragma unroll
    for (int r = 0; r < 4; ++r) {
      const bool active = s < len[r];
      const int tt = reverse ? len[r] - 1 - s : s;
      const int b = b0 + quad * 4 + r;
      const float* row = gi + ((long)tt * B + b) * (G * H);
#pragma unroll
      for (int nt = 0; nt < NTW; ++nt) {
        const int u = wave * (H / NW) + nt * 16 + l15;
#pragma unroll
        for (int gt = 0; gt < G; ++gt) dst[gt][nt][r] = active ? row[gt * H + u] : 0.f;
      }
    }
  };
  auto fetch = [&](int s) { fetch_into(s, gx); };
  fetch(0);

#ifdef RNN_SEQ_DBG_TIME
  long long f_m = 0, f_g = 0, f_b = 0;
#endif
  for (int s = 0; s < Lt; ++s) {
#ifdef RNN_SEQ_DBG_TIME
    const long long f_t0 = clock64();
#endif
    const int cur = s & 1;
    f32x4 acc[G][NTW];
    float xn[NTW][4];
#pragma unroll
    for (int r = 0; r < 4; ++r)
#pragma unroll
      for (int nt = 0; nt < NTW; ++nt)
#pragma unroll
        for (int gt = 0; gt < G; ++gt) {
          const float x = gx[gt][nt][r];
          if (KIND == 1 && gt == 2) {
            xn[nt][r] = x;
            acc[gt][nt][r] = bias[gt][nt];
          } else {
            acc[gt][nt][r] = x + bias[gt][nt];
          }
        }
#pragma unroll
    for (int ks = 0; ks < KS; ++ks) {
      bf16x8 a[3];
#pragma unroll
      for (int q = 0; q < 3; ++q)
        a[q] = *reinterpret_cast<const bf16x8*>(&h_pl[cur][q][l15][32 * ks + 8 * quad]);
      Planes3 wl;
      const bool from_lds = KL > 0 && ks >= KS - KL;
      if (from_lds) {
#pragma unroll
        for (int q = 0; q < 3; ++q) wl.p[q] = w_lds[KL > 0 ? ks - (KS - KL) : 0][q][tid];
      }
#pragma unroll
      for (int q = 0; q < 6; ++q)
#pragma unroll
        for (int gt = 0; gt < G; ++gt)
#pragma unroll
          for (int nt = 0; nt < NTW; ++nt) {
            const bf16x8 wb = (from_lds && gt == G - 1 && nt == 0) ? wl.p[X3_PB[q]]
                                                                   : wp[gt][nt][ks].p[X3_PB[q]];
            acc[gt][nt] = __builtin_amdgcn_mfma_f32_16x16x32_bf16(a[X3_PA[q]], wb, acc[gt][nt], 0, 0, 0);
          }
    }
    fetch(s + 1);
#ifdef RNN_SEQ_DBG_TIME
    const long long f_t1 = clock64();
#endif
#pragma unroll
    for (int r = 0; r < 4; ++r) {
      const bool active = s < len[r];
      const int tt = reverse ? len[r] - 1 - s : s;
      const int b = b0 + quad * 4 + r;
      const int row_i = quad * 4 + r;
#pragma unroll
      for (int nt = 0; nt < NTW; ++nt) {
        const int u = wave * (H / NW) + nt * 16 + l15;
        float hnew;
        if (KIND == 0) {
          const float ig = sigm(acc[0][nt][r]), fg = sigm(acc[1][nt][r]);
          const float gg = tanh_fast(acc[2][nt][r]), og = sigm(acc[3][nt][r]);
          const float cn = fg * creg[nt][r] + ig * gg;
          hnew = og * tanh_fast(cn);
          if (active) {
            creg[nt][r] = cn;
            if (p.gates[d]) {
              float* gs = p.gates[d] + ((long)tt * B + b) * (G * H);
              gs[u] = ig;
              gs[H + u] = fg;
              gs[2 * H + u] = gg;
              gs[3 * H + u] = og;
              p.aux[d][((long)tt * B + b) * H + u] = cn;
            }
          }
        } else {
          const float rg = sigm(acc[0][nt][r]), zg = sigm(acc[1][nt][r]);
          const float hn = acc[2][nt][r];
          const float ng = tanh_fast(xn[nt][r] + rg * hn);
          hnew = (1.f - zg) * ng + zg * hreg[nt][r];
          if (active && p.gates[d]) {
            float* gs = p.gates[d] + ((long)tt * B + b) * (G * H);
            gs[u] = rg;
            gs[H + u] = zg;
            gs[2 * H + u] = ng;
            p.aux[d][((long)tt * B + b) * H + u] = hn;
          }
        }
        if (active) {
          hreg[nt][r] = hnew;
          p.out[d][((long)tt * B + b) * H + u] = hnew;
          if (p.seq[d]) p.seq[d][(long)tt * p.seq_st + (long)b * p.seq_sb + u] = hnew;
        }
        unsigned short hw[3];
        split_scalar(hreg[nt][r], hw);
#pragma unroll
        for (int q = 0; q < 3; ++q) h_pl[cur ^ 1][q][row_i][u] = hw[q];
      }
    }
#ifdef RNN_SEQ_DBG_TIME
    const long long f_t2 = clock64();
#endif
    __syncthreads();
#ifdef RNN_SEQ_DBG_TIME
    const long long f_t3 = clock64();
    f_m += f_t1 - f_t0;
    f_g += f_t2 - f_t1;
    f_b += f_t3 - f_t2;
#endif
  }
#ifdef RNN_SEQ_DBG_TIME
  if (blockIdx.x == 0 && blockIdx.y == 0 && (tid == 0 || tid == 64 * (NW - 1)))
    printf("rnn_seq_fwd wave %d: %d steps; per step: init+fetch+reads+MFMA %lld, gates+stores+LDS write %lld, "
           "barrier %lld cycles\n", wave, Lt, f_m / Lt, f_g / Lt, f_b / Lt);
#endif
#pragma unroll
  for (int r = 0; r < 4; ++r) {
    const int b = b0 + quad * 4 + r;
    if (b < B)
#pragma unroll
      for (int nt = 0; nt < NTW; ++nt)
        p.h_final[d][(long)b * H + wave * (H / NW) + nt * 16 + l15] = hreg[nt][r];
  }
}

template <int KIND, int H, int NW>
__global__ __launch_bounds__(NW * 64) void rnn_seq_bwd_kernel(RnnSeqParams p) {
  constexpr int G = KIND == 0 ? 4 : 3;
  constexpr int NTW = H / (NW * 16);
  constexpr int GH = G * H;
  constexpr int KS = GH / 32;
  constexpr int LDGB = GH + 16;
  static_assert(NTW >= 1, "units per wave");
  __shared__ __attribute__((aligned(16))) unsigned short dg_pl[3][16][LDGB];
  constexpr int KL = (KIND == 0 && H == 128) ? 4 : 0;
  __shared__ __attribute__((aligned(16))) bf16x8 w_lds[KL > 0 ? KL : 1][3][NW * 64];
  const int d = blockIdx.y;
  const int b0 = blockIdx.x * 16;
  const int tid = threadIdx.x, lane = tid & 63, wave = tid >> 6;
  const int l15 = lane & 15, quad = lane >> 4;
  const bool reverse = d == 1;
  const float* __restrict__ WT = p.w_hh[d];
  const int B = p.B, L = p.L;
  if (p.self_zero) {
    zero_tails<NW * 64>(p.dgi[d], (long)B * GH, GH, GH, p.lengths, b0, B, L, tid);
    if (KIND == 1) zero_tails<NW * 64>(p.dgh[d], (long)B * GH, GH, GH, p.lengths, b0, B, L, tid);
  }

  int len[4];
#pragma unroll
  for (int r = 0; r < 4; ++r) {
    const int b = b0 + quad * 4 + r;
    len[r] = b < B ? p.lengths[b] : 0;
  }
  int Lt = max(max(len[0], len[1]), max(len[2], len[3]));
  Lt = max(Lt, __shfl_xor(Lt, 16, 64));
  Lt = max(Lt, __shfl_xor(Lt, 32, 64));
  Lt = min(Lt, L);
  Planes3 wt[NTW][KS];
#pragma unroll
  for (int nt = 0; nt < NTW; ++nt) {
    const int n = wave * (H / NW) + nt * 16 + l15;
#pragma unroll
    for (int ks = 0; ks < KS; ++ks) {
      f32x4 lo4, hi4;
      if (p.w_plain) {
        const float* wk = WT + (long)(32 * ks + 8 * quad) * H + n;
#pragma unroll
        for (int i = 0; i < 4; ++i) {
          lo4[i] = wk[(long)i * H];
          hi4[i] = wk[(long)(i + 4) * H];
        }
      } else {
        const float* w8 = WT + (long)n * GH + 32 * ks + 8 * quad;
        lo4 = *reinterpret_cast<const f32x4*>(w8);
        hi4 = *reinterpret_cast<const f32x4*>(w8 + 4);
      }
      wt[nt][ks] = split_planes(lo4, hi4);
      if (KL > 0 && nt == 0 && ks >= KS - KL) {
#pragma unroll
        for (int q = 0; q < 3; ++q) w_lds[ks - (KS - KL)][q][tid] = wt[nt][ks].p[q];
      }
    }
  }
  float dh[NTW][4], dc[NTW][4];
#pragma unroll
  for (int nt = 0; nt < NTW; ++nt)
#pragma unroll
    for (int r = 0; r < 4; ++r) {
      const int b = b0 + quad * 4 + r;
      const int u = wave * (H / NW) + nt * 16 + l15;
      dh[nt][r] = (p.dh_final[d] && b < B) ? p.dh_final[d][(long)b * H + u] : 0.f;
      dc[nt][r] = 0.f;
    }

  float pg[G][NTW][4], pa[NTW][4], pa_prev[NTW][4], pd[NTW][4];
  auto fetch_row = [&](int s, int r, float (&g_)[G][NTW][4], float (&a_)[NTW][4], float (&d_)[NTW][4]) {
    {
      const bool active = s >= 0 && s < len[r];
      const int tt = reverse ? len[r] - 1 - s : s;
      const int b = b0 + quad * 4 + r;
      const long base = ((long)tt * B + b);
#pragma unroll
      for (int nt = 0; nt < NTW; ++nt) {
        const int u = wave * (H / NW) + nt * 16 + l15;
#pragma unroll
        for (int gt = 0; gt < G; ++gt) g_[gt][nt][r] = active ? p.gates[d][base * GH + gt * H + u] : 0.f;
        a_[nt][r] = active ? p.aux[d][base * H + u] : 0.f;
        d_[nt][r] = (active && p.dout[d]) ? p.dout[d][base * H + u] : 0.f;
      }
    }
  };
  auto fetch = [&](int s, float (&g_)[G][NTW][4], float (&a_)[NTW][4], float (&d_)[NTW][4]) {
#pragma unroll
    for (int r = 0; r < 4; ++r) fetch_row(s, r, g_, a_, d_);
  };
  auto fetch_prev_row = [&](int s, int r, float (&a_)[NTW][4]) {
    {
      const bool active = s >= 0 && s < len[r];
      const int tt = reverse ? len[r] - 1 - s : s;
      const int b = b0 + quad * 4 + r;
#pragma unroll
      for (int nt = 0; nt < NTW; ++nt) {
        const int u = wave * (H / NW) + nt * 16 + l15;
        const float* src = KIND == 0 ? p.aux[d] : p.out[d];
        a_[nt][r] = active ? src[((long)tt * B + b) * H + u] : 0.f;
      }
    }
  };
  auto fetch_prev = [&](int s, float (&a_)[NTW][4]) {
#pragma unroll
    for (int r = 0; r < 4; ++r) fetch_prev_row(s, r, a_);
  };
  fetch(Lt - 1, pg, pa, pd);
  fetch_prev(Lt - 2, pa_prev);

#ifdef RNN_SEQ_DBG_TIME
  long long d_a = 0, d_b1 = 0, d_m = 0, d_b2 = 0;
#endif
  for (int s = Lt - 1; s >= 0; --s) {
#ifdef RNN_SEQ_DBG_TIME
    const long long d_t0 = clock64();
#endif
    float keep_z[NTW][4];
    float cg[G][NTW][4], ca[NTW][4], cprev[NTW][4], cd[NTW][4];
#pragma unroll
    for (int r = 0; r < 4; ++r)
#pragma unroll
      for (int nt = 0; nt < NTW; ++nt) {
#pragma unroll
        for (int gt = 0; gt < G; ++gt) cg[gt][nt][r] = pg[gt][nt][r];
        ca[nt][r] = pa[nt][r];
        cprev[nt][r] = pa_prev[nt][r];
        cd[nt][r] = pd[nt][r];
      }
    fetch(s - 1, pg, pa, pd);
    fetch_prev(s - 2, pa_prev);
#pragma unroll
    for (int r = 0; r < 4; ++r) {
      const bool active = s < len[r];
      const int tt = reverse ? len[r] - 1 - s : s;
      const int b = b0 + quad * 4 + r;
      const int row_i = quad * 4 + r;
      const long base = ((long)tt * B + b);
#pragma unroll
      for (int nt = 0; nt < NTW; ++nt) {
        const int u = wave * (H / NW) + nt * 16 + l15;
        float dpre[G];
#pragma unroll
        for (int gt = 0; gt < G; ++gt) dpre[gt] = 0.f;
        float dgh_n = 0.f;
        keep_z[nt][r] = 0.f;
        if (active) {
          const float dht = dh[nt][r] + cd[nt][r];
          if (KIND == 0) {
            const float ig = cg[0][nt][r], fg = cg[1][nt][r], gg = cg[2][nt][r], og = cg[3][nt][r];
            const float c = ca[nt][r];
            const float cp = cprev[nt][r];
            const float tc = tanh_fast(c);
            const float dct = dc[nt][r] + dht * og * (1.f - tc * tc);
            dpre[0] = dct * gg * ig * (1.f - ig);
            dpre[1] = dct * cp * fg * (1.f - fg);
            dpre[2] = dct * ig * (1.f - gg * gg);
            dpre[3] = dht * tc * og * (1.f - og);
            dc[nt][r] = dct * fg;
          } else {
            const float rg = cg[0][nt][r], zg = cg[1][nt][r], ng = cg[2][nt][r];
            const float hn = ca[nt][r];
            const float hp = cprev[nt][r];
            const float dn = dht * (1.f - zg);
            const float dz = dht * (hp - ng);
            const float dnp = dn * (1.f - ng * ng);
            dpre[0] = dnp * hn * rg * (1.f - rg);
            dpre[1] = dz * zg * (1.f - zg);
            dpre[2] = dnp;
            dgh_n = dnp * rg;
            keep_z[nt][r] = dht * zg;
          }
          float* dgi = p.dgi[d] + base * GH;
#pragma unroll
          for (int gt = 0; gt < G; ++gt) dgi[gt * H + u] = dpre[gt];
          if (KIND == 1) {
            float* dgh = p.dgh[d] + base * GH;
            dgh[u] = dpre[0];
            dgh[H + u] = dpre[1];
            dgh[2 * H + u] = dgh_n;
          }
        }
#pragma unroll
        for (int gt = 0; gt < G; ++gt) {
          unsigned short dw[3];
          split_scalar((KIND == 1 && gt == 2) ? dgh_n : dpre[gt], dw);
#pragma unroll
          for (int q = 0; q < 3; ++q) dg_pl[q][row_i][gt * H + u] = dw[q];
        }
      }
    }
#ifdef RNN_SEQ_DBG_TIME
    const long long d_t1 = clock64();
#endif
    __syncthreads();
#ifdef RNN_SEQ_DBG_TIME
    const long long d_t2 = clock64();
#endif
    f32x4 acc[NTW];
#pragma unroll
    for (int nt = 0; nt < NTW; ++nt) acc[nt] = f32x4{0.f, 0.f, 0.f, 0.f};
#pragma unroll
    for (int ks = 0; ks < KS; ++ks) {
      bf16x8 a[3];
#pragma unroll
      for (int q = 0; q < 3; ++q)
        a[q] = *reinterpret_cast<const bf16x8*>(&dg_pl[q][l15][32 * ks + 8 * quad]);
      Planes3 wl;
      const bool from_lds = KL > 0 && ks >= KS - KL;
      if (from_lds) {
#pragma unroll
        for (int q = 0; q < 3; ++q) wl.p[q] = w_lds[KL > 0 ? ks - (KS - KL) : 0][q][tid];
      }
#pragma unroll
      for (int q = 0; q < 6; ++q)
#pragma unroll
        for (int nt = 0; nt < NTW; ++nt) {
          const bf16x8 wb = (from_lds && nt == 0) ? wl.p[X3_PB[q]] : wt[nt][ks].p[X3_PB[q]];
          acc[nt] = __builtin_amdgcn_mfma_f32_16x16x32_bf16(a[X3_PA[q]], wb, acc[nt], 0, 0, 0);
        }
    }
#pragma unroll
    for (int r = 0; r < 4; ++r) {
      const bool active = s < len[r];
      if (active)
#pragma unroll
        for (int nt = 0; nt < NTW; ++nt) dh[nt][r] = acc[nt][r] + keep_z[nt][r];
    }
#ifdef RNN_SEQ_DBG_TIME
    const long long d_t3 = clock64();
#endif
    __syncthreads();
#ifdef RNN_SEQ_DBG_TIME
    const long long d_t4 = clock64();
    d_a += d_t1 - d_t0;
    d_b1 += d_t2 - d_t1;
    d_m += d_t3 - d_t2;
    d_b2 += d_t4 - d_t3;
#endif
  }
#ifdef RNN_SEQ_DBG_TIME
  if (blockIdx.x == 0 && blockIdx.y == 0 && (tid == 0 || tid == 64 * (NW - 1)))
    printf("rnn_seq_bwd wave %d: %d steps; per step: gates+LDS write %lld, barrier %lld, reads+MFMA %lld, "
           "barrier %lld cycles\n", wave, Lt, d_a / Lt, d_b1 / Lt, d_m / Lt, d_b2 / Lt);
#endif
}

template <int KIND>
int launch_fwd(const RnnSeqParams& p, int H, int dirs, hipStream_t s) {
  dim3 grid(ceil_div(p.B, 16), dirs);
  if (H == 64)
    hipLaunchKernelGGL((rnn_seq_fwd_kernel<KIND, 64, 4>), grid, dim3(256), 0, s, p);
  else if (H == 128)
    hipLaunchKernelGGL((rnn_seq_fwd_kernel<KIND, 128, 8>), grid, dim3(512), 0, s, p);
  else
    return 1;
  return 0;
}
template <int KIND>
int launch_bwd(const RnnSeqParams& p, int H, int dirs, hipStream_t s) {
  dim3 grid(ceil_div(p.B, 16), dirs);
  if (H == 64)
    hipLaunchKernelGGL((rnn_seq_bwd_kernel<KIND, 64, 4>), grid, dim3(256), 0, s, p);
  else if (H == 128)
    hipLaunchKernelGGL((rnn_seq_bwd_kernel<KIND, 128, 8>), grid, dim3(512), 0, s, p);
  else
    return 1;
  return 0;
}

}

extern "C" int vlnce_rnn_seq_supported(int kind, int H) {
  return (kind == 0 || kind == 1) && (H == 64 || H == 128);
}

extern "C" int vlnce_rnn_seq_fwd(int kind, int dirs, const float* const* gi,
                                 const float* const* w_hh, const float* const* b_hh,
                                 const int* lengths, float* const* out, float* const* h_final,
                                 float* const* gates_save, float* const* aux_save, int B, int L,
                                 int H, vlnce_stream_t stream) {
  VLNCE_CHECK_ARG(gi && w_hh && b_hh && lengths && out && h_final, "rnn_seq_fwd: null argument");
  VLNCE_CHECK_ARG(dirs == 1 || dirs == 2, "rnn_seq_fwd: dirs must be 1 or 2");
  VLNCE_CHECK_ARG(vlnce_rnn_seq_supported(kind, H), "rnn_seq_fwd: unsupported kind/H (%d,%d)", kind, H);
  VLNCE_CHECK_ARG(B > 0 && L > 0, "rnn_seq_fwd: bad shape");
  RnnSeqParams p{};
  for (int d = 0; d < dirs; ++d) {
    p.gi[d] = gi[d];
    p.w_hh[d] = w_hh[d];
    p.b_hh[d] = b_hh[d];
    p.out[d] = out[d];
    p.h_final[d] = h_final[d];
    p.gates[d] = gates_save ? gates_save[d] : nullptr;
    p.aux[d] = aux_save ? aux_save[d] : nullptr;
    VLNCE_CHECK_ARG((p.gates[d] == nullptr) == (p.aux[d] == nullptr),
                    "rnn_seq_fwd: gates_save and aux_save come together");
  }
  p.lengths = lengths;
  p.B = B;
  p.L = L;
  hipStream_t s = reinterpret_cast<hipStream_t>(stream);
  const int rc = kind == 0 ? launch_fwd<0>(p, H, dirs, s) : launch_fwd<1>(p, H, dirs, s);
  VLNCE_CHECK_ARG(rc == 0, "rnn_seq_fwd: no kernel for H=%d", H);
  VLNCE_CHECK_LAUNCH("rnn_seq_fwd");
  return 0;
}

extern "C" int vlnce_rnn_seq_bwd(int kind, int dirs, const float* const* w_hh_t,
                                 const int* lengths, const float* const* out,
                                 const float* const* gates_save, const float* const* aux_save,
                                 const float* const* dout, const float* const* dh_final,
                                 float* const* dgi, float* const* dgh, int B, int L, int H,
                                 vlnce_stream_t stream) {
  VLNCE_CHECK_ARG(w_hh_t && lengths && out && gates_save && aux_save && dgi,
                  "rnn_seq_bwd: null argument");
  VLNCE_CHECK_ARG(dirs == 1 || dirs == 2, "rnn_seq_bwd: dirs must be 1 or 2");
  VLNCE_CHECK_ARG(vlnce_rnn_seq_supported(kind, H), "rnn_seq_bwd: unsupported kind/H (%d,%d)", kind, H);
  VLNCE_CHECK_ARG(kind == 0 || dgh, "rnn_seq_bwd: GRU needs dgh");
  RnnSeqParams p{};
  for (int d = 0; d < dirs; ++d) {
    p.w_hh[d] = w_hh_t[d];
    p.out[d] = const_cast<float*>(out[d]);
    p.gates[d] = const_cast<float*>(gates_save[d]);
    p.aux[d] = const_cast<float*>(aux_save[d]);
    p.dout[d] = dout ? dout[d] : nullptr;
    p.dh_final[d] = dh_final ? dh_final[d] : nullptr;
    p.dgi[d] = dgi[d];
    p.dgh[d] = dgh ? dgh[d] : nullptr;
  }
  p.lengths = lengths;
  p.B = B;
  p.L = L;
  hipStream_t s = reinterpret_cast<hipStream_t>(stream);
  const int rc = kind == 0 ? launch_bwd<0>(p, H, dirs, s) : launch_bwd<1>(p, H, dirs, s);
  VLNCE_CHECK_ARG(rc == 0, "rnn_seq_bwd: no kernel for H=%d", H);
  VLNCE_CHECK_LAUNCH("rnn_seq_bwd");
  return 0;
}


extern "C" int vlnce_rnn_seq_fwd2(int kind, int dirs, const float* const* gi,
                                  const float* const* w_hh, const float* const* b_hh,
                                  const int* lengths, float* const* out_tm, float* seq,
                                  long seq_st, long seq_sb, float* const* h_final,
                                  float* const* gates_save, float* const* aux_save, int B, int L,
                                  int H, vlnce_stream_t stream) {
  VLNCE_CHECK_ARG(gi && w_hh && b_hh && lengths && out_tm && h_final, "rnn_seq_fwd2: null argument");
  VLNCE_CHECK_ARG(dirs == 1 || dirs == 2, "rnn_seq_fwd2: dirs must be 1 or 2");
  VLNCE_CHECK_ARG(vlnce_rnn_seq_supported(kind, H), "rnn_seq_fwd2: unsupported kind/H (%d,%d)", kind, H);
  VLNCE_CHECK_ARG(B > 0 && L > 0, "rnn_seq_fwd2: bad shape");
  VLNCE_CHECK_ARG(!seq || (seq_st > 0 && seq_sb > 0), "rnn_seq_fwd2: seq needs its strides");
  RnnSeqParams p{};
  for (int d = 0; d < dirs; ++d) {
    p.gi[d] = gi[d];
    p.w_hh[d] = w_hh[d];
    p.b_hh[d] = b_hh[d];
    p.out[d] = out_tm[d];
    p.seq[d] = seq ? seq + (long)d * H : nullptr;
    p.h_final[d] = h_final[d];
    p.gates[d] = gates_save ? gates_save[d] : nullptr;
    p.aux[d] = aux_save ? aux_save[d] : nullptr;
    VLNCE_CHECK_ARG((p.gates[d] == nullptr) == (p.aux[d] == nullptr),
                    "rnn_seq_fwd2: gates_save and aux_save come together");
  }
  p.seq_st = seq_st;
  p.seq_sb = seq_sb;
  p.self_zero = 1;
  p.lengths = lengths;
  p.B = B;
  p.L = L;
  hipStream_t s = reinterpret_cast<hipStream_t>(stream);
  const int rc = kind == 0 ? launch_fwd<0>(p, H, dirs, s) : launch_fwd<1>(p, H, dirs, s);
  VLNCE_CHECK_ARG(rc == 0, "rnn_seq_fwd2: no kernel for H=%d", H);
  VLNCE_CHECK_LAUNCH("rnn_seq_fwd2");
  return 0;
}

extern "C" int vlnce_rnn_seq_bwd2(int kind, int dirs, const float* const* w_hh, const int* lengths,
                                  const float* const* out_tm, const float* const* gates_save,
                                  const float* const* aux_save, const float* dseq, long dseq_st,
                                  long dseq_sb, float* dout_ws, const float* const* dh_final,
                                  float* const* dgi, float* const* dgh, int B, int L, int H,
                                  vlnce_stream_t stream) {
  VLNCE_CHECK_ARG(w_hh && lengths && out_tm && gates_save && aux_save && dgi,
                  "rnn_seq_bwd2: null argument");
  VLNCE_CHECK_ARG(dirs == 1 || dirs == 2, "rnn_seq_bwd2: dirs must be 1 or 2");
  VLNCE_CHECK_ARG(vlnce_rnn_seq_supported(kind, H), "rnn_seq_bwd2: unsupported kind/H (%d,%d)", kind, H);
  VLNCE_CHECK_ARG(kind == 0 || dgh, "rnn_seq_bwd2: GRU needs dgh");
  VLNCE_CHECK_ARG(!dseq || (dseq_st > 0 && dseq_sb > 0), "rnn_seq_bwd2: dseq needs its strides");
  VLNCE_CHECK_ARG(!dseq || dout_ws, "rnn_seq_bwd2: dseq needs the dirs*L*B*H workspace");
  hipStream_t s = reinterpret_cast<hipStream_t>(stream);
  if (dseq) {
    const long n4 = (long)dirs * L * B * (H / 4);
    const int grid = (int)((n4 + 255) / 256 > 2048 ? 2048 : (n4 + 255) / 256);
    hipLaunchKernelGGL(dseq_to_time_major_kernel, dim3(grid), dim3(256), 0, s, dseq, dseq_st, dseq_sb,
                       dout_ws, dirs, L, B, H);
    VLNCE_CHECK_LAUNCH("rnn_seq_bwd2 (output gradient to time-major)");
  }
  RnnSeqParams p{};
  for (int d = 0; d < dirs; ++d) {
    p.w_hh[d] = w_hh[d];
    p.out[d] = const_cast<float*>(out_tm[d]);
    p.gates[d] = const_cast<float*>(gates_save[d]);
    p.aux[d] = const_cast<float*>(aux_save[d]);
    p.dout[d] = dseq ? dout_ws + (long)d * L * B * H : nullptr;
    p.dh_final[d] = dh_final ? dh_final[d] : nullptr;
    p.dgi[d] = dgi[d];
    p.dgh[d] = dgh ? dgh[d] : nullptr;
  }
  p.self_zero = 1;
  p.w_plain = 1;
  p.lengths = lengths;
  p.B = B;
  p.L = L;
  const int rc = kind == 0 ? launch_bwd<0>(p, H, dirs, s) : launch_bwd<1>(p, H, dirs, s);
  VLNCE_CHECK_ARG(rc == 0, "rnn_seq_bwd2: no kernel for H=%d", H);
  VLNCE_CHECK_LAUNCH("rnn_seq_bwd2");
  return 0;
}

extern "C" int vlnce_rnn_seq_wgrad(int kind, int dirs, int first_dir, const float* const* dgi,
                                   const float* const* dgh, const float* const* out_tm,
                                   const float* x_tm, int ldx, int E, const float* const* w_ih,
                                   float* const* dw_ih, float* const* dw_hh, float* const* db_ih,
                                   float* const* db_hh, float* dx_tm, int B, int L, int H,
                                   vlnce_stream_t stream) {
  VLNCE_CHECK_ARG(dgi && out_tm && x_tm && dw_ih && dw_hh && db_ih && db_hh,
                  "rnn_seq_wgrad: null argument");
  VLNCE_CHECK_ARG(dirs == 1 || dirs == 2, "rnn_seq_wgrad: dirs must be 1 or 2");
  VLNCE_CHECK_ARG((first_dir == 0 || first_dir == 1) && first_dir + dirs <= 2,
                  "rnn_seq_wgrad: first_dir + dirs must stay within the two directions");
  VLNCE_CHECK_ARG(kind == 0 || dgh, "rnn_seq_wgrad: GRU needs dgh");
  VLNCE_CHECK_ARG(!dx_tm || w_ih, "rnn_seq_wgrad: dx_tm needs w_ih");
  const int GH = (kind == 0 ? 4 : 3) * H;
  const long rows = (long)L * B;
  VLNCE_CHECK_ARG(B > 0 && L > 0 && E > 0 && ldx >= E && rows < 0x7fffffffL, "rnn_seq_wgrad: bad shape");
  hipStream_t s = reinterpret_cast<hipStream_t>(stream);
  for (int d = 0; d < dirs; ++d) {
    const float* dGh = kind == 1 ? dgh[d] : dgi[d];
    if (L > 1) {
      const bool reverse = first_dir + d == 1;
      const float* dG_s = reverse ? dGh : dGh + (long)B * GH;
      const float* h_s = reverse ? out_tm[d] + (long)B * H : out_tm[d];
      int rc = vlnce_gemm(dG_s, GH, 1, h_s, H, 1, dw_hh[d], H, GH, H, (int)((long)(L - 1) * B), nullptr, stream);
      if (rc != 0) return rc;
    } else {
      vlnce_zero(dw_hh[d], GH, H, H, s);
    }
    int rc = vlnce_colsum(dGh, GH, (int)rows, GH, db_hh[d], 0, stream);
    if (rc != 0) return rc;
    rc = vlnce_gemm(dgi[d], GH, 1, x_tm, ldx, 1, dw_ih[d], E, GH, E, (int)rows, nullptr, stream);
    if (rc != 0) return rc;
    if (db_ih[d] != db_hh[d]) {
      rc = vlnce_colsum(dgi[d], GH, (int)rows, GH, db_ih[d], 0, stream);
      if (rc != 0) return rc;
    }
    if (dx_tm) {
      vlnce_epilogue e{};
      e.accumulate = d > 0;
      rc = vlnce_gemm(dgi[d], GH, 0, w_ih[d], E, 1, dx_tm, E, (int)rows, E, GH, &e, stream);
      if (rc != 0) return rc;
    }
  }
  return 0;
}
```

Baseline: 8429.

## Add 4/8-row RNN sequence workgroups and fold strided dseq into backward

Templates the sequence RNN forward and backward kernels on rows per workgroup (4, 8 or 16). At small batch it picks fewer rows per workgroup so more workgroups cover the CUs, trading MFMA row utilisation for parallelism. The backward kernel can read the output gradient directly through strides, skipping the separate time-major transpose kernel when fewer rows are used. Training forward stays at 16 rows by default, and a few gate updates are rewritten as FMAs.

New measurement: 8290. 1.7% lower.

```diff
diff --git a/include/vlnce_hip.h b/include/vlnce_hip.h
--- a/include/vlnce_hip.h
+++ b/include/vlnce_hip.h
@@ -338,6 +338,8 @@
                        float* dout_ws ,
                        const float* const* dh_final, float* const* dgi, float* const* dgh,
                        int B, int L, int H, vlnce_stream_t stream);
+int vlnce_rnn_seq_last_rows(void);
+int vlnce_rnn_seq_last_workgroups(void);
 int vlnce_rnn_seq_wgrad(int kind, int dirs, int first_dir, const float* const* dgi, const float* const* dgh,
                         const float* const* out_tm, const float* x_tm, int ldx, int E,
                         const float* const* w_ih, float* const* dw_ih, float* const* dw_hh,
diff --git a/vln-ce_amd/_lib.py b/vln-ce_amd/_lib.py
--- a/vln-ce_amd/_lib.py
+++ b/vln-ce_amd/_lib.py
@@ -196,6 +196,8 @@
     "vlnce_maxpool3x3s2_bwd": (_I, [_P, _P, _P, _I, _I, _I, _I, _I, _I, _P]),
     "vlnce_adaptive_avgpool_bwd": (_I, [_P, _P, _I, _I, _I, _I, _I, _I, _P]),
     "vlnce_rnn_seq_supported": (_I, [_I, _I]),
+    "vlnce_rnn_seq_last_rows": (_I, []),
+    "vlnce_rnn_seq_last_workgroups": (_I, []),
     "vlnce_rnn_seq_fwd": (_I, [_I, _I, _P, _P, _P, _P, _P, _P, _P, _P, _I, _I, _I, _P]),
     "vlnce_rnn_seq_bwd": (_I, [_I, _I, _P, _P, _P, _P, _P, _P, _P, _P, _P, _I, _I, _I, _P]),
     "vlnce_option_count": (_I, []),
@@ -306,7 +308,7 @@
 
     name = "hip"
 
-    ABI = 150
+    ABI = 151
 
     def __init__(self, path=LIB_PATH):
         self.dll = load_cdll(path)
@@ -321,7 +323,7 @@
 
     OPTION_NAMES = ("conv_math", "p3", "p3_tile", "s3", "u3", "u3_waves", "x3_tile", "igemm_tile",
                     "igemm_nobuf", "igemm_no_splitk", "wgrad_tile", "rollout_one_xcd", "m3", "r3",
-                    "s3_wgs")
+                    "s3_wgs", "rnn_rows")
 
     def _options_from_env(self):
         for name in self.OPTION_NAMES:
@@ -877,6 +879,9 @@
     def rnn_seq_supported(self, kind, H):
         return bool(self.dll.vlnce_rnn_seq_supported(kind, H))
 
+    def rnn_seq_last_launch(self):
+        return int(self.dll.vlnce_rnn_seq_last_rows()), int(self.dll.vlnce_rnn_seq_last_workgroups())
+
     def rnn_seq_fwd(self, kind, dirs, gi, w_hh, b_hh, lengths, out, h_final, gates_save, aux_save,
                     B, Lm, H):
         pa = self._parr
diff --git a/vln-ce_amd/csrc/api.cpp b/vln-ce_amd/csrc/api.cpp
--- a/vln-ce_amd/csrc/api.cpp
+++ b/vln-ce_amd/csrc/api.cpp
@@ -16,7 +16,7 @@
 }
 
 extern "C" const char* vlnce_last_error(void) { return g_err; }
-extern "C" int vlnce_version(void) { return 150; }
+extern "C" int vlnce_version(void) { return 151; }
 
 namespace {
 struct OptDef {
@@ -27,10 +27,10 @@
     {"conv_math", 2},   {"p3", 2},          {"p3_tile", 0},         {"s3", 1},
     {"u3", 1},          {"u3_waves", 8},    {"x3_tile", 0},         {"igemm_tile", 0},
     {"igemm_nobuf", 0}, {"igemm_no_splitk", 0}, {"wgrad_tile", 64}, {"rollout_one_xcd", 0},
-    {"m3", 1},          {"r3", 1},          {"s3_wgs", 0},
+    {"m3", 1},          {"r3", 1},          {"s3_wgs", 0},          {"rnn_rows", 0},
 };
 std::atomic<int> g_opt[VLNCE_OPT_COUNT] = {
-    {2}, {2}, {0}, {1}, {1}, {8}, {0}, {0}, {0}, {0}, {64}, {0}, {1}, {1}, {0},
+    {2}, {2}, {0}, {1}, {1}, {8}, {0}, {0}, {0}, {0}, {64}, {0}, {1}, {1}, {0}, {0},
 };
 int opt_index(const char* name) {
   if (name)
diff --git a/vln-ce_amd/csrc/common_opts.h b/vln-ce_amd/csrc/common_opts.h
--- a/vln-ce_amd/csrc/common_opts.h
+++ b/vln-ce_amd/csrc/common_opts.h
@@ -19,6 +19,7 @@
   VLNCE_OPT_M3,
   VLNCE_OPT_R3,
   VLNCE_OPT_S3_WGS,
+  VLNCE_OPT_RNN_ROWS,
   VLNCE_OPT_COUNT
 };
 int vlnce_opt(int id);
diff --git a/vln-ce_amd/csrc/rnn_seq.hip b/vln-ce_amd/csrc/rnn_seq.hip
--- a/vln-ce_amd/csrc/rnn_seq.hip
+++ b/vln-ce_amd/csrc/rnn_seq.hip
@@ -20,6 +20,7 @@
   long seq_st, seq_sb;
   int self_zero;
   int w_plain;
+  long dout_st, dout_sb;
 };
 
 __global__ __launch_bounds__(256) void dseq_to_time_major_kernel(const float* __restrict__ dseq, long st,
@@ -40,11 +41,11 @@
   }
 }
 
-template <int NT>
+template <int NT, int ROWS>
 __device__ __forceinline__ void zero_tails(float* __restrict__ base, long st, long sb, int width,
                                            const int* __restrict__ lengths, int b0, int B, int L,
                                            int tid) {
-  for (int r = 0; r < 16; ++r) {
+  for (int r = 0; r < ROWS; ++r) {
     const int b = b0 + r;
     if (b >= B) break;
     const int lb = min(max(lengths[b], 0), L);
@@ -100,36 +101,42 @@
 constexpr int X3_PA[6] = {2, 0, 1, 1, 0, 0};
 constexpr int X3_PB[6] = {0, 2, 1, 0, 1, 0};
 
-template <int KIND, int H, int NW>
+template <int KIND, int H, int NW, int ROWS>
 __global__ __launch_bounds__(NW * 64) void rnn_seq_fwd_kernel(RnnSeqParams p) {
   constexpr int G = KIND == 0 ? 4 : 3;
   constexpr int NTW = H / (NW * 16);
   static_assert(NTW >= 1, "units per wave");
+  static_assert(ROWS == 16 || ROWS == 8 || ROWS == 4, "rows per workgroup");
+  constexpr int RL = ROWS / 4;
+  constexpr int TR = ROWS == 16 ? 16 : ROWS + 1;
   constexpr int KS = H / 32;
   constexpr int LDHB = H + 16;
-  __shared__ __attribute__((aligned(16))) unsigned short h_pl[2][3][16][LDHB];
-  constexpr int KL = (KIND == 0 && H == 128) ? 3 : 0;
+  __shared__ __attribute__((aligned(16))) unsigned short h_pl[2][3][TR][LDHB];
+  constexpr int KL = (KIND == 0 && H == 128 && ROWS >= 8) ? 3 : 0;
   __shared__ __attribute__((aligned(16))) bf16x8 w_lds[KL > 0 ? KL : 1][3][NW * 64];
   const int d = blockIdx.y;
-  const int b0 = blockIdx.x * 16;
+  const int b0 = blockIdx.x * ROWS;
   const int tid = threadIdx.x, lane = tid & 63, wave = tid >> 6;
   const int l15 = lane & 15, quad = lane >> 4;
+  const int a_row = (ROWS == 16 || (l15 & 3) < RL) ? (l15 >> 2) * RL + (l15 & 3) : ROWS;
   const bool reverse = d == 1;
   const float* __restrict__ gi = p.gi[d];
   const float* __restrict__ W = p.w_hh[d];
   const int B = p.B, L = p.L;
   if (p.self_zero) {
-    zero_tails<NW * 64>(p.out[d], (long)B * H, H, H, p.lengths, b0, B, L, tid);
-    if (p.seq[d]) zero_tails<NW * 64>(p.seq[d], p.seq_st, p.seq_sb, H, p.lengths, b0, B, L, tid);
-  }
-
-  int len[4];
-#pragma unroll
-  for (int r = 0; r < 4; ++r) {
-    const int b = b0 + quad * 4 + r;
+    zero_tails<NW * 64, ROWS>(p.out[d], (long)B * H, H, H, p.lengths, b0, B, L, tid);
+    if (p.seq[d]) zero_tails<NW * 64, ROWS>(p.seq[d], p.seq_st, p.seq_sb, H, p.lengths, b0, B, L, tid);
+  }
+
+  int len[RL];
+#pragma unroll
+  for (int r = 0; r < RL; ++r) {
+    const int b = b0 + quad * RL + r;
     len[r] = b < B ? p.lengths[b] : 0;
   }
-  int Lt = max(max(len[0], len[1]), max(len[2], len[3]));
+  int Lt = len[0];
+#pragma unroll
+  for (int r = 1; r < RL; ++r) Lt = max(Lt, len[r]);
   Lt = max(Lt, __shfl_xor(Lt, 16, 64));
   Lt = max(Lt, __shfl_xor(Lt, 32, 64));
   Lt = min(Lt, L);
@@ -152,21 +159,21 @@
         }
       }
     }
-  float hreg[NTW][4], creg[NTW][4];
+  float hreg[NTW][RL], creg[NTW][RL];
 #pragma unroll
   for (int nt = 0; nt < NTW; ++nt)
 #pragma unroll
-    for (int r = 0; r < 4; ++r) hreg[nt][r] = creg[nt][r] = 0.f;
-  for (int i = tid; i < 3 * 16 * LDHB; i += NW * 64) (&h_pl[0][0][0][0])[i] = 0;
+    for (int r = 0; r < RL; ++r) hreg[nt][r] = creg[nt][r] = 0.f;
+  for (int i = tid; i < (ROWS == 16 ? 3 : 6) * TR * LDHB; i += NW * 64) (&h_pl[0][0][0][0])[i] = 0;
   __syncthreads();
 
-  float gx[G][NTW][4];
-  auto fetch_into = [&](int s, float (&dst)[G][NTW][4]) {
-#pragma unroll
-    for (int r = 0; r < 4; ++r) {
+  float gx[G][NTW][RL];
+  auto fetch_into = [&](int s, float (&dst)[G][NTW][RL]) {
+#pragma unroll
+    for (int r = 0; r < RL; ++r) {
       const bool active = s < len[r];
       const int tt = reverse ? len[r] - 1 - s : s;
-      const int b = b0 + quad * 4 + r;
+      const int b = b0 + quad * RL + r;
       const float* row = gi + ((long)tt * B + b) * (G * H);
 #pragma unroll
       for (int nt = 0; nt < NTW; ++nt) {
@@ -188,9 +195,15 @@
 #endif
     const int cur = s & 1;
     f32x4 acc[G][NTW];
-    float xn[NTW][4];
-#pragma unroll
-    for (int r = 0; r < 4; ++r)
+    float xn[NTW][RL];
+    if (RL < 4) {
+#pragma unroll
+      for (int gt = 0; gt < G; ++gt)
+#pragma unroll
+        for (int nt = 0; nt < NTW; ++nt) acc[gt][nt] = f32x4{0.f, 0.f, 0.f, 0.f};
+    }
+#pragma unroll
+    for (int r = 0; r < RL; ++r)
 #pragma unroll
       for (int nt = 0; nt < NTW; ++nt)
 #pragma unroll
@@ -208,7 +221,7 @@
       bf16x8 a[3];
 #pragma unroll
       for (int q = 0; q < 3; ++q)
-        a[q] = *reinterpret_cast<const bf16x8*>(&h_pl[cur][q][l15][32 * ks + 8 * quad]);
+        a[q] = *reinterpret_cast<const bf16x8*>(&h_pl[cur][q][a_row][32 * ks + 8 * quad]);
       Planes3 wl;
       const bool from_lds = KL > 0 && ks >= KS - KL;
       if (from_lds) {
@@ -231,11 +244,11 @@
     const long long f_t1 = clock64();
 #endif
 #pragma unroll
-    for (int r = 0; r < 4; ++r) {
+    for (int r = 0; r < RL; ++r) {
       const bool active = s < len[r];
       const int tt = reverse ? len[r] - 1 - s : s;
-      const int b = b0 + quad * 4 + r;
-      const int row_i = quad * 4 + r;
+      const int b = b0 + quad * RL + r;
+      const int row_i = quad * RL + r;
 #pragma unroll
       for (int nt = 0; nt < NTW; ++nt) {
         const int u = wave * (H / NW) + nt * 16 + l15;
@@ -243,7 +256,7 @@
         if (KIND == 0) {
           const float ig = sigm(acc[0][nt][r]), fg = sigm(acc[1][nt][r]);
           const float gg = tanh_fast(acc[2][nt][r]), og = sigm(acc[3][nt][r]);
-          const float cn = fg * creg[nt][r] + ig * gg;
+          const float cn = __builtin_fmaf(ig, gg, fg * creg[nt][r]);
           hnew = og * tanh_fast(cn);
           if (active) {
             creg[nt][r] = cn;
@@ -260,7 +273,8 @@
           const float rg = sigm(acc[0][nt][r]), zg = sigm(acc[1][nt][r]);
           const float hn = acc[2][nt][r];
           const float ng = tanh_fast(xn[nt][r] + rg * hn);
-          hnew = (1.f - zg) * ng + zg * hreg[nt][r];
+          hnew = H == 128 ? __builtin_fmaf(zg, hreg[nt][r], (1.f - zg) * ng)
+                          : __builtin_fmaf(1.f - zg, ng, zg * hreg[nt][r]);
           if (active && p.gates[d]) {
             float* gs = p.gates[d] + ((long)tt * B + b) * (G * H);
             gs[u] = rg;
@@ -293,12 +307,12 @@
   }
 #ifdef RNN_SEQ_DBG_TIME
   if (blockIdx.x == 0 && blockIdx.y == 0 && (tid == 0 || tid == 64 * (NW - 1)))
-    printf("rnn_seq_fwd wave %d: %d steps; per step: init+fetch+reads+MFMA %lld, gates+stores+LDS write %lld, "
-           "barrier %lld cycles\n", wave, Lt, f_m / Lt, f_g / Lt, f_b / Lt);
-#endif
-#pragma unroll
-  for (int r = 0; r < 4; ++r) {
-    const int b = b0 + quad * 4 + r;
+    printf("rnn_seq_fwd ROWS %d wave %d: %d steps; per step: init+fetch+reads+MFMA %lld, gates+stores+LDS write %lld, "
+           "barrier %lld cycles\n", ROWS, wave, Lt, f_m / Lt, f_g / Lt, f_b / Lt);
+#endif
+#pragma unroll
+  for (int r = 0; r < RL; ++r) {
+    const int b = b0 + quad * RL + r;
     if (b < B)
 #pragma unroll
       for (int nt = 0; nt < NTW; ++nt)
@@ -306,7 +320,7 @@
   }
 }
 
-template <int KIND, int H, int NW>
+template <int KIND, int H, int NW, int ROWS, bool DS>
 __global__ __launch_bounds__(NW * 64) void rnn_seq_bwd_kernel(RnnSeqParams p) {
   constexpr int G = KIND == 0 ? 4 : 3;
   constexpr int NTW = H / (NW * 16);
@@ -314,28 +328,34 @@
   constexpr int KS = GH / 32;
   constexpr int LDGB = GH + 16;
   static_assert(NTW >= 1, "units per wave");
-  __shared__ __attribute__((aligned(16))) unsigned short dg_pl[3][16][LDGB];
+  static_assert(ROWS == 16 || ROWS == 8 || ROWS == 4, "rows per workgroup");
+  constexpr int RL = ROWS / 4;
+  constexpr int TR = ROWS == 16 ? 16 : ROWS + 1;
+  __shared__ __attribute__((aligned(16))) unsigned short dg_pl[3][TR][LDGB];
   constexpr int KL = (KIND == 0 && H == 128) ? 4 : 0;
   __shared__ __attribute__((aligned(16))) bf16x8 w_lds[KL > 0 ? KL : 1][3][NW * 64];
   const int d = blockIdx.y;
-  const int b0 = blockIdx.x * 16;
+  const int b0 = blockIdx.x * ROWS;
   const int tid = threadIdx.x, lane = tid & 63, wave = tid >> 6;
   const int l15 = lane & 15, quad = lane >> 4;
+  const int a_row = (ROWS == 16 || (l15 & 3) < RL) ? (l15 >> 2) * RL + (l15 & 3) : ROWS;
   const bool reverse = d == 1;
   const float* __restrict__ WT = p.w_hh[d];
   const int B = p.B, L = p.L;
   if (p.self_zero) {
-    zero_tails<NW * 64>(p.dgi[d], (long)B * GH, GH, GH, p.lengths, b0, B, L, tid);
-    if (KIND == 1) zero_tails<NW * 64>(p.dgh[d], (long)B * GH, GH, GH, p.lengths, b0, B, L, tid);
-  }
-
-  int len[4];
-#pragma unroll
-  for (int r = 0; r < 4; ++r) {
-    const int b = b0 + quad * 4 + r;
+    zero_tails<NW * 64, ROWS>(p.dgi[d], (long)B * GH, GH, GH, p.lengths, b0, B, L, tid);
+    if (KIND == 1) zero_tails<NW * 64, ROWS>(p.dgh[d], (long)B * GH, GH, GH, p.lengths, b0, B, L, tid);
+  }
+
+  int len[RL];
+#pragma unroll
+  for (int r = 0; r < RL; ++r) {
+    const int b = b0 + quad * RL + r;
     len[r] = b < B ? p.lengths[b] : 0;
   }
-  int Lt = max(max(len[0], len[1]), max(len[2], len[3]));
+  int Lt = len[0];
+#pragma unroll
+  for (int r = 1; r < RL; ++r) Lt = max(Lt, len[r]);
   Lt = max(Lt, __shfl_xor(Lt, 16, 64));
   Lt = max(Lt, __shfl_xor(Lt, 32, 64));
   Lt = min(Lt, L);
@@ -365,23 +385,23 @@
       }
     }
   }
-  float dh[NTW][4], dc[NTW][4];
+  float dh[NTW][RL], dc[NTW][RL];
 #pragma unroll
   for (int nt = 0; nt < NTW; ++nt)
 #pragma unroll
-    for (int r = 0; r < 4; ++r) {
-      const int b = b0 + quad * 4 + r;
+    for (int r = 0; r < RL; ++r) {
+      const int b = b0 + quad * RL + r;
       const int u = wave * (H / NW) + nt * 16 + l15;
       dh[nt][r] = (p.dh_final[d] && b < B) ? p.dh_final[d][(long)b * H + u] : 0.f;
       dc[nt][r] = 0.f;
     }
 
-  float pg[G][NTW][4], pa[NTW][4], pa_prev[NTW][4], pd[NTW][4];
-  auto fetch_row = [&](int s, int r, float (&g_)[G][NTW][4], float (&a_)[NTW][4], float (&d_)[NTW][4]) {
+  float pg[G][NTW][RL], pa[NTW][RL], pa_prev[NTW][RL], pd[NTW][RL];
+  auto fetch_row = [&](int s, int r, float (&g_)[G][NTW][RL], float (&a_)[NTW][RL], float (&d_)[NTW][RL]) {
     {
       const bool active = s >= 0 && s < len[r];
       const int tt = reverse ? len[r] - 1 - s : s;
-      const int b = b0 + quad * 4 + r;
+      const int b = b0 + quad * RL + r;
       const long base = ((long)tt * B + b);
 #pragma unroll
       for (int nt = 0; nt < NTW; ++nt) {
@@ -389,19 +409,22 @@
 #pragma unroll
         for (int gt = 0; gt < G; ++gt) g_[gt][nt][r] = active ? p.gates[d][base * GH + gt * H + u] : 0.f;
         a_[nt][r] = active ? p.aux[d][base * H + u] : 0.f;
-        d_[nt][r] = (active && p.dout[d]) ? p.dout[d][base * H + u] : 0.f;
+        if (DS)
+          d_[nt][r] = (active && p.dout[d]) ? p.dout[d][(long)tt * p.dout_st + (long)b * p.dout_sb + u] : 0.f;
+        else
+          d_[nt][r] = (active && p.dout[d]) ? p.dout[d][base * H + u] : 0.f;
       }
     }
   };
-  auto fetch = [&](int s, float (&g_)[G][NTW][4], float (&a_)[NTW][4], float (&d_)[NTW][4]) {
-#pragma unroll
-    for (int r = 0; r < 4; ++r) fetch_row(s, r, g_, a_, d_);
+  auto fetch = [&](int s, float (&g_)[G][NTW][RL], float (&a_)[NTW][RL], float (&d_)[NTW][RL]) {
+#pragma unroll
+    for (int r = 0; r < RL; ++r) fetch_row(s, r, g_, a_, d_);
   };
-  auto fetch_prev_row = [&](int s, int r, float (&a_)[NTW][4]) {
+  auto fetch_prev_row = [&](int s, int r, float (&a_)[NTW][RL]) {
     {
       const bool active = s >= 0 && s < len[r];
       const int tt = reverse ? len[r] - 1 - s : s;
-      const int b = b0 + quad * 4 + r;
+      const int b = b0 + quad * RL + r;
 #pragma unroll
       for (int nt = 0; nt < NTW; ++nt) {
         const int u = wave * (H / NW) + nt * 16 + l15;
@@ -410,10 +433,13 @@
       }
     }
   };
-  auto fetch_prev = [&](int s, float (&a_)[NTW][4]) {
-#pragma unroll
-    for (int r = 0; r < 4; ++r) fetch_prev_row(s, r, a_);
+  auto fetch_prev = [&](int s, float (&a_)[NTW][RL]) {
+#pragma unroll
+    for (int r = 0; r < RL; ++r) fetch_prev_row(s, r, a_);
   };
+  if (ROWS < 16) {
+    for (int i = tid; i < 3 * LDGB; i += NW * 64) dg_pl[i / LDGB][ROWS][i % LDGB] = 0;
+  }
   fetch(Lt - 1, pg, pa, pd);
   fetch_prev(Lt - 2, pa_prev);
 
@@ -424,10 +450,10 @@
 #ifdef RNN_SEQ_DBG_TIME
     const long long d_t0 = clock64();
 #endif
-    float keep_z[NTW][4];
-    float cg[G][NTW][4], ca[NTW][4], cprev[NTW][4], cd[NTW][4];
-#pragma unroll
-    for (int r = 0; r < 4; ++r)
+    float keep_z[NTW][RL];
+    float cg[G][NTW][RL], ca[NTW][RL], cprev[NTW][RL], cd[NTW][RL];
+#pragma unroll
+    for (int r = 0; r < RL; ++r)
 #pragma unroll
       for (int nt = 0; nt < NTW; ++nt) {
 #pragma unroll
@@ -439,11 +465,11 @@
     fetch(s - 1, pg, pa, pd);
     fetch_prev(s - 2, pa_prev);
 #pragma unroll
-    for (int r = 0; r < 4; ++r) {
+    for (int r = 0; r < RL; ++r) {
       const bool active = s < len[r];
       const int tt = reverse ? len[r] - 1 - s : s;
-      const int b = b0 + quad * 4 + r;
-      const int row_i = quad * 4 + r;
+      const int b = b0 + quad * RL + r;
+      const int row_i = quad * RL + r;
       const long base = ((long)tt * B + b);
 #pragma unroll
       for (int nt = 0; nt < NTW; ++nt) {
@@ -513,7 +539,7 @@
       bf16x8 a[3];
 #pragma unroll
       for (int q = 0; q < 3; ++q)
-        a[q] = *reinterpret_cast<const bf16x8*>(&dg_pl[q][l15][32 * ks + 8 * quad]);
+        a[q] = *reinterpret_cast<const bf16x8*>(&dg_pl[q][a_row][32 * ks + 8 * quad]);
       Planes3 wl;
       const bool from_lds = KL > 0 && ks >= KS - KL;
       if (from_lds) {
@@ -529,7 +555,7 @@
         }
     }
 #pragma unroll
-    for (int r = 0; r < 4; ++r) {
+    for (int r = 0; r < RL; ++r) {
       const bool active = s < len[r];
       if (active)
 #pragma unroll
@@ -549,32 +575,72 @@
   }
 #ifdef RNN_SEQ_DBG_TIME
   if (blockIdx.x == 0 && blockIdx.y == 0 && (tid == 0 || tid == 64 * (NW - 1)))
-    printf("rnn_seq_bwd wave %d: %d steps; per step: gates+LDS write %lld, barrier %lld, reads+MFMA %lld, "
-           "barrier %lld cycles\n", wave, Lt, d_a / Lt, d_b1 / Lt, d_m / Lt, d_b2 / Lt);
-#endif
-}
-
+    printf("rnn_seq_bwd ROWS %d wave %d: %d steps; per step: gates+LDS write %lld, barrier %lld, reads+MFMA %lld, "
+           "barrier %lld cycles\n", ROWS, wave, Lt, d_a / Lt, d_b1 / Lt, d_m / Lt, d_b2 / Lt);
+#endif
+}
+
+int device_cus() {
+  static int cus[16];
+  int dev = 0;
+  if (hipGetDevice(&dev) != hipSuccess || dev < 0 || dev >= 16) return 256;
+  if (cus[dev] == 0) {
+    int c = 0;
+    if (hipDeviceGetAttribute(&c, hipDeviceAttributeMultiprocessorCount, dev) != hipSuccess || c <= 0) c = 256;
+    cus[dev] = c;
+  }
+  return cus[dev];
+}
+thread_local int g_last_rows = 0, g_last_wgs = 0;
+int pick_rows(int B, int dirs, bool train_fwd) {
+  const int o = vlnce_opt(VLNCE_OPT_RNN_ROWS);
+  if (o == 4 || o == 8 || o == 16) return o;
+  if (train_fwd && o != 1) return 16;
+  const int cus = device_cus();
+  for (int rows = 4; rows < 16; rows *= 2)
+    if ((long)ceil_div(B, rows) * dirs <= cus) return rows;
+  return 16;
+}
+
+template <int KIND, int ROWS>
+int launch_fwd_rows(const RnnSeqParams& p, int H, int dirs, hipStream_t s) {
+  dim3 grid(ceil_div(p.B, ROWS), dirs);
+  if (H == 64)
+    hipLaunchKernelGGL((rnn_seq_fwd_kernel<KIND, 64, 4, ROWS>), grid, dim3(256), 0, s, p);
+  else if (H == 128)
+    hipLaunchKernelGGL((rnn_seq_fwd_kernel<KIND, 128, 8, ROWS>), grid, dim3(512), 0, s, p);
+  else
+    return 1;
+  g_last_rows = ROWS;
+  g_last_wgs = (int)(grid.x * grid.y);
+  return 0;
+}
 template <int KIND>
 int launch_fwd(const RnnSeqParams& p, int H, int dirs, hipStream_t s) {
-  dim3 grid(ceil_div(p.B, 16), dirs);
+  const int rows = pick_rows(p.B, dirs, p.gates[0] != nullptr);
+  return rows == 4 ? launch_fwd_rows<KIND, 4>(p, H, dirs, s)
+       : rows == 8 ? launch_fwd_rows<KIND, 8>(p, H, dirs, s)
+                   : launch_fwd_rows<KIND, 16>(p, H, dirs, s);
+}
+template <int KIND, int ROWS>
+int launch_bwd_rows(const RnnSeqParams& p, int H, int dirs, hipStream_t s) {
+  constexpr bool DS = ROWS < 16;
+  dim3 grid(ceil_div(p.B, ROWS), dirs);
   if (H == 64)
-    hipLaunchKernelGGL((rnn_seq_fwd_kernel<KIND, 64, 4>), grid, dim3(256), 0, s, p);
+    hipLaunchKernelGGL((rnn_seq_bwd_kernel<KIND, 64, 4, ROWS, DS>), grid, dim3(256), 0, s, p);
   else if (H == 128)
-    hipLaunchKernelGGL((rnn_seq_fwd_kernel<KIND, 128, 8>), grid, dim3(512), 0, s, p);
+    hipLaunchKernelGGL((rnn_seq_bwd_kernel<KIND, 128, 8, ROWS, DS>), grid, dim3(512), 0, s, p);
   else
     return 1;
+  g_last_rows = ROWS;
+  g_last_wgs = (int)(grid.x * grid.y);
   return 0;
 }
 template <int KIND>
-int launch_bwd(const RnnSeqParams& p, int H, int dirs, hipStream_t s) {
-  dim3 grid(ceil_div(p.B, 16), dirs);
-  if (H == 64)
-    hipLaunchKernelGGL((rnn_seq_bwd_kernel<KIND, 64, 4>), grid, dim3(256), 0, s, p);
-  else if (H == 128)
-    hipLaunchKernelGGL((rnn_seq_bwd_kernel<KIND, 128, 8>), grid, dim3(512), 0, s, p);
-  else
-    return 1;
-  return 0;
+int launch_bwd(const RnnSeqParams& p, int rows, int H, int dirs, hipStream_t s) {
+  return rows == 4 ? launch_bwd_rows<KIND, 4>(p, H, dirs, s)
+       : rows == 8 ? launch_bwd_rows<KIND, 8>(p, H, dirs, s)
+                   : launch_bwd_rows<KIND, 16>(p, H, dirs, s);
 }
 
 }
@@ -582,6 +648,9 @@
 extern "C" int vlnce_rnn_seq_supported(int kind, int H) {
   return (kind == 0 || kind == 1) && (H == 64 || H == 128);
 }
+
+extern "C" int vlnce_rnn_seq_last_rows(void) { return g_last_rows; }
+extern "C" int vlnce_rnn_seq_last_workgroups(void) { return g_last_wgs; }
 
 extern "C" int vlnce_rnn_seq_fwd(int kind, int dirs, const float* const* gi,
                                  const float* const* w_hh, const float* const* b_hh,
@@ -639,8 +708,11 @@
   p.lengths = lengths;
   p.B = B;
   p.L = L;
+  p.dout_st = (long)B * H;
+  p.dout_sb = H;
   hipStream_t s = reinterpret_cast<hipStream_t>(stream);
-  const int rc = kind == 0 ? launch_bwd<0>(p, H, dirs, s) : launch_bwd<1>(p, H, dirs, s);
+  const int rows = pick_rows(B, dirs, false);
+  const int rc = kind == 0 ? launch_bwd<0>(p, rows, H, dirs, s) : launch_bwd<1>(p, rows, H, dirs, s);
   VLNCE_CHECK_ARG(rc == 0, "rnn_seq_bwd: no kernel for H=%d", H);
   VLNCE_CHECK_LAUNCH("rnn_seq_bwd");
   return 0;
@@ -697,8 +769,11 @@
   VLNCE_CHECK_ARG(kind == 0 || dgh, "rnn_seq_bwd2: GRU needs dgh");
   VLNCE_CHECK_ARG(!dseq || (dseq_st > 0 && dseq_sb > 0), "rnn_seq_bwd2: dseq needs its strides");
   VLNCE_CHECK_ARG(!dseq || dout_ws, "rnn_seq_bwd2: dseq needs the dirs*L*B*H workspace");
+  VLNCE_CHECK_ARG(B > 0 && L > 0, "rnn_seq_bwd2: bad shape");
   hipStream_t s = reinterpret_cast<hipStream_t>(stream);
-  if (dseq) {
+  const int rows = pick_rows(B, dirs, false);
+  const bool folded = rows < 16;
+  if (dseq && !folded) {
     const long n4 = (long)dirs * L * B * (H / 4);
     const int grid = (int)((n4 + 255) / 256 > 2048 ? 2048 : (n4 + 255) / 256);
     hipLaunchKernelGGL(dseq_to_time_major_kernel, dim3(grid), dim3(256), 0, s, dseq, dseq_st, dseq_sb,
@@ -711,17 +786,19 @@
     p.out[d] = const_cast<float*>(out_tm[d]);
     p.gates[d] = const_cast<float*>(gates_save[d]);
     p.aux[d] = const_cast<float*>(aux_save[d]);
-    p.dout[d] = dseq ? dout_ws + (long)d * L * B * H : nullptr;
+    p.dout[d] = !dseq ? nullptr : folded ? dseq + (long)d * H : dout_ws + (long)d * L * B * H;
     p.dh_final[d] = dh_final ? dh_final[d] : nullptr;
     p.dgi[d] = dgi[d];
     p.dgh[d] = dgh ? dgh[d] : nullptr;
   }
+  p.dout_st = folded ? dseq_st : (long)B * H;
+  p.dout_sb = folded ? dseq_sb : H;
   p.self_zero = 1;
   p.w_plain = 1;
   p.lengths = lengths;
   p.B = B;
   p.L = L;
-  const int rc = kind == 0 ? launch_bwd<0>(p, H, dirs, s) : launch_bwd<1>(p, H, dirs, s);
+  const int rc = kind == 0 ? launch_bwd<0>(p, rows, H, dirs, s) : launch_bwd<1>(p, rows, H, dirs, s);
   VLNCE_CHECK_ARG(rc == 0, "rnn_seq_bwd2: no kernel for H=%d", H);
   VLNCE_CHECK_LAUNCH("rnn_seq_bwd2");
   return 0;
```
